# life-ufes/multimodal-model-skin-lesion-classifier

Measured on AMD Instinct MI355X. Metric: images/sec fwd+bwd, ResNet-50+crossattention bs=256, higher is better.
Workload: dtype bf16; 1 GPU; ResNet-50 + one-hot(20) + crossattention, 224x224, train step incl. Adam; per_gpu_batch=256, global_batch=256, parallelism=dp1, weights=random init (torchvision / timm / transformers layouts), unfreeze_weights=unfrozen_weights, linear_dtype=fp32

## Files before the change

include/mmskin.h:

```cpp
#ifndef MMSKIN_H
#define MMSKIN_H
#include <stdint.h>

#ifdef __cplusplus
extern "C" {
#endif

#define MMSKIN_F32 0
#define MMSKIN_BF16 1

const char* mmskin_last_error(void);
int mmskin_version(void);

typedef struct mmskin_backbone* mmskin_backbone_t;
int mmskin_backbone_create(const char* arch, int batch, int height, int width, int dtype, mmskin_backbone_t* out);
void mmskin_backbone_destroy(mmskin_backbone_t h);
int mmskin_backbone_num_tensors(mmskin_backbone_t h, int kind );
int mmskin_backbone_tensor_info(mmskin_backbone_t h, int kind, int index, char* name, int name_cap,
                                int64_t* offset, int64_t* numel, int* ndim, int64_t* shape4);
int64_t mmskin_backbone_param_numel(mmskin_backbone_t h);
int64_t mmskin_backbone_buffer_numel(mmskin_backbone_t h);
int64_t mmskin_backbone_workspace_bytes(mmskin_backbone_t h);
int mmskin_backbone_feature_dim(mmskin_backbone_t h);
int mmskin_backbone_feature_hw(mmskin_backbone_t h, int* out_h, int* out_w);
int mmskin_backbone_num_units(mmskin_backbone_t h);
int mmskin_backbone_unit_info(mmskin_backbone_t h, int index, char* name, int name_cap, int64_t* info12);
int mmskin_backbone_profile_enable(mmskin_backbone_t h, int on);
int mmskin_backbone_profile_read(mmskin_backbone_t h, double* ms7, double* flops7, double* bytes7, int64_t* launches7);
int mmskin_backbone_forward(mmskin_backbone_t h, const float* image_nchw, const float* params, float* buffers,
                            void* workspace, float* features, int training, void* stream);
int mmskin_backbone_forward_u8(mmskin_backbone_t h, const uint8_t* image_nhwc, const float* mean_std6, const float* params,
                               float* buffers, void* workspace, float* features, int training, void* stream);
int mmskin_backbone_set_option(mmskin_backbone_t h, const char* key, int value);
int mmskin_backbone_set_pointer(mmskin_backbone_t h, const char* key, const void* device_ptr);
int mmskin_backbone_num_grad_segments(mmskin_backbone_t h, int* count);
int mmskin_backbone_grad_segment(mmskin_backbone_t h, int index, int64_t* offset, int64_t* numel);
int mmskin_backbone_wait_grad_segment(mmskin_backbone_t h, int index, void* stream);
int mmskin_backbone_last_conv_shape(mmskin_backbone_t h, int* C, int* OH, int* OW);
int mmskin_backbone_last_conv_export(mmskin_backbone_t h, const void* workspace, float* x_nchw, void* stream);
int mmskin_backbone_last_conv_grad(mmskin_backbone_t h, const float* dfeatures, const void* workspace, float* dx_nchw,
                                   void* stream);
int mmskin_backbone_backward(mmskin_backbone_t h, const float* dfeatures, const float* params, void* workspace,
                             float* param_grads, void* stream);

int64_t mmskin_conv2d_workspace_bytes(int N, int Cin, int H, int W, int Cout, int kh, int kw, int stride, int pad);
int mmskin_conv2d_forward(const float* x, const float* w, float* y, int N, int Cin, int H, int W, int Cout, int kh,
                          int kw, int stride, int pad, int dtype, void* workspace, void* stream);
int mmskin_conv2d_backward(const float* dy, const float* x, const float* w, float* dx, float* dw, int N, int Cin,
                           int H, int W, int Cout, int kh, int kw, int stride, int pad, int dtype, void* workspace,
                           void* stream);
int mmskin_conv2d_dgrad_fused_rows(int N, int Cin, int H, int W, int Cout, int kh, int kw, int stride, int pad);
int mmskin_conv2d_dgrad_fused(const float* dy, const float* w, const float* xc, const float* scale, const float* shift, float* dz,
                              float* partial, int* rows_written, int N, int Cin, int H, int W, int Cout, int kh, int kw, int stride,
                              int pad, void* workspace, void* stream);
int64_t mmskin_conv3x3_c64_launches(void);
int64_t mmskin_stem7x7_launches(void);
double mmskin_conv2d_time(int N, int Cin, int H, int W, int Cout, int kh, int kw, int stride, int pad, int dtype,
                          int iters, void* workspace, void* stream);
double mmskin_conv2d_dgrad_time(int N, int Cin, int H, int W, int Cout, int kh, int kw, int stride, int pad, int dtype,
                                int iters, void* workspace, void* stream);
double mmskin_conv2d_wgrad_time(int N, int Cin, int H, int W, int Cout, int kh, int kw, int stride, int pad, int dtype,
                                int iters, void* workspace, void* stream);
int64_t mmskin_conv_pipe_launches(void);
int64_t mmskin_wgrad_ring_launches(void);
int64_t mmskin_wgrad3_ring_launches(void);
int64_t mmskin_abn_workspace_bytes(int N, int Cw, int C4, int H, int W);
int mmskin_abn_backward(const float* g, const float* y, const float* w, const float* cA, const float* cB, const float* cC, int N, int Cw,
                        int C4, int H, int W, float* dy, float* dw, void* workspace, void* stream);
int mmskin_abn_backward_kept_gram(const float* g, const float* y, const float* w, const float* cA, const float* cB, const float* cC, int N,
                                  int Cw, int C4, int H, int W, float* dy, float* dw, void* workspace, void* stream);
int mmskin_conv1x1_gram_stats(const float* y, const float* w, int N, int Cw, int C4, int H, int W, float* stat_sum, float* stat_sq,
                              void* workspace, void* stream);
int64_t mmskin_batchnorm_workspace_bytes(int N, int C, int H, int W);
int mmskin_batchnorm_forward(const float* x, const float* gamma, const float* beta, float* running_mean,
                             float* running_var, float* y, float* save_mean, float* save_invstd, int N, int C, int H,
                             int W, float eps, float momentum, int relu, int dtype, void* workspace, void* stream);
int mmskin_batchnorm_backward(const float* dy, const float* x, const float* gamma, const float* beta,
                              const float* save_mean, const float* save_invstd, float* dx, float* dgamma, float* dbeta,
                              int N, int C, int H, int W, int relu, int dtype, void* workspace, void* stream);
int64_t mmskin_stem_workspace_bytes(int N, int H, int W);
int mmskin_stem_forward(const float* x, const float* w, const float* gamma, const float* beta, float* y, int N, int H,
                        int W, float eps, int dtype, void* workspace, void* stream);
int mmskin_stem_backward(const float* dy, const float* x, const float* w, const float* gamma, const float* beta,
                         float* dw, float* dgamma, float* dbeta, int N, int H, int W, float eps, int dtype,
                         void* workspace, void* stream);

int mmskin_linear_forward(const float* x, const float* w, const float* b, float* y, int M, int K, int N, int relu,
                          void* stream);
int mmskin_linear_backward(const float* dy, const float* x, const float* w, const float* y_relu, float* dy_scratch,
                           float* dx, float* dw, float* db, int M, int K, int N, void* stream);
int mmskin_linear_gelu_backward(const float* dh, const float* x, const float* w, const float* z, float* dy_scratch, float* dx, float* dw,
                                float* db, int M, int K, int N, void* stream);
int mmskin_linear_x16_pitch(int M, int K, int N);
enum { MMSKIN_LINEAR_SMALL = 0, MMSKIN_LINEAR_BIG_F32 = 1, MMSKIN_LINEAR_BIG_BF16 = 2, MMSKIN_LINEAR_PADDED_BF16 = 3 };
int mmskin_linear_route(int M, int K, int N);
int mmskin_linear_forward_keep(const float* x, const float* w, const float* b, const float* res, float* y, void* x16_keep, int M, int K,
                               int N, int relu, void* stream);
int mmskin_linear_backward_keep(const float* dy, const void* x16, const float* w, const float* y_relu, const float* z_gelu, float* dy_scratch,
                                float* dx, float* dw, float* db, int M, int K, int N, void* stream);
int mmskin_gelu_forward_bf16(const float* z, void* h16, int64_t rows, int cols, int cols_pad, void* stream);
int mmskin_linear_forward_x16(const void* x16, const float* w, const float* b, const float* res, float* y, int M, int K, int N, int relu,
                              void* stream);
int mmskin_star_relu_forward_bf16(const float* z, const float* s, const float* b, void* h16, int64_t rows, int cols, int cols_pad,
                                  void* stream);
int mmskin_linear_star_relu_backward_keep(const float* dh, const void* x16, const float* w, const float* z, const float* s, float* dsb,
                                          float* dx, float* dw, float* db, int M, int K, int N, void* stream);
int mmskin_star_relu_forward(const float* z, const float* s, const float* b, float* y, int64_t n, void* stream);
int mmskin_star_relu_backward(const float* dy, const float* z, const float* s, float* dz, float* dsb, int64_t n, void* stream);
int mmskin_layernorm_forward(const float* x, const float* g, const float* b, float* y, float* mean, float* rstd,
                             int M, int N, float eps, int relu, void* stream);
int mmskin_layernorm_backward(const float* dy, const float* x, const float* g, const float* b, const float* mean,
                              const float* rstd, float* dx, float* dg, float* db, int M, int N, int relu, void* stream);
int mmskin_sigmoid_gate_forward(const float* z, const float* v, float* out, int64_t n, void* stream);
int mmskin_sigmoid_gate_backward(const float* dout, const float* z, const float* v, float* dz, float* dv, int64_t n,
                                 void* stream);
int mmskin_gated_mix_forward(const float* z, const float* a, const float* q, float* out, int64_t n, void* stream);
int mmskin_gated_mix_backward(const float* dout, const float* z, const float* a, const float* q, float* dz, float* da,
                              float* dq, int64_t n, void* stream);
int mmskin_metablock_gate_forward(const float* V, const float* t1, const float* t2, float* out, int64_t n, void* stream);
int mmskin_metablock_gate_backward(const float* dout, const float* V, const float* t1, const float* t2, float* dV,
                                   float* dt1, float* dt2, int64_t n, void* stream);
int mmskin_adam_step(float* p, const float* g, float* m, float* v, int64_t n, double lr, double beta1, double beta2, double eps,
                     double weight_decay, int64_t step, void* stream);
int mmskin_dropout_forward(const float* x, float* y, uint8_t* mask, int64_t n, float p, uint64_t seed,
                           uint64_t offset, void* stream);
int mmskin_attn_dropout_forward(const float* x, float* y, uint8_t* mask, int64_t n, int L, float p, uint64_t seed, uint64_t offset,
                                void* stream);
int mmskin_dropout_backward(const float* dy, const uint8_t* mask, float* dx, int64_t n, float p, void* stream);
int mmskin_concat2_forward(const float* a, const float* b, float* out, int M, int Na, int Nb, void* stream);
int mmskin_concat2_backward(const float* dout, float* da, float* db, int M, int Na, int Nb, void* stream);
int mmskin_attention_forward(const float* q, const float* k, const float* v, float* o, float* p, int B, int H, int L,
                             int Dh, float drop_p, uint64_t seed, uint64_t offset, void* stream);
int mmskin_attention_backward(const float* dO, const float* q, const float* k, const float* v, const float* p,
                              float* dq, float* dk, float* dv, int B, int H, int L, int Dh, float drop_p,
                              uint64_t seed, uint64_t offset, void* stream);
int mmskin_mdnet_fuse_forward(const float* feat, const float* z, const float* t1, const float* t2, float* pooled,
                              int64_t NC, int HW, void* stream);
int mmskin_mdnet_fuse_backward(const float* dpooled, const float* feat, const float* z, const float* t1, const float* t2,
                               float* dfeat , float* dz, float* dt1, float* dt2, int64_t NC, int HW,
                               void* stream);
int mmskin_bmm(const float* a, const float* b, float* c, int batch, int M, int N, int K, int64_t sam, int64_t sak, int64_t sab,
               int64_t sbn, int64_t sbk, int64_t sbb, int64_t ldc, int64_t scb, void* stream);
int mmskin_softmax_forward(const float* x, const float* mask_add, const float* bias ,
                           float* y, int64_t rows, int L, int64_t rows_per_batch, float scale,
                           int causal , void* stream);
int mmskin_softmax_backward(const float* dy, const float* y, float* dx, int64_t rows, int L, float scale, void* stream);
int mmskin_colsum(const float* x, float* out, int M, int N, void* stream);
int mmskin_scale_add_forward(const float* x, const float* b, const float* gamma, float* y, int64_t n, int C, void* stream);
int mmskin_scale_mul(const float* dy, const float* v, float* out, int64_t n, int C, int per_channel, void* stream);
int mmskin_token_mean_forward(const float* x, float* out, int B, int L, int E, int start, void* stream);
int mmskin_token_mean_backward(const float* dout, float* dx, int B, int L, int E, int start, void* stream);
int mmskin_flash_attention_forward(const void* q, const void* k, const void* v, const float* mask_add, const float* bias,
                                   void* o, float* lse, int B, int H, int L, int Dh, const int64_t* strides12, int io_dtype,
                                   float scale, int causal, float drop_p, uint64_t seed, uint64_t offset, void* stream);
int mmskin_flash_attention_backward(const float* q, const float* k, const float* v, const float* o, const float* dout, const float* lse,
                                    const float* mask_add, const float* bias, const float* biasT, float* delta, float* dq, float* dk,
                                    float* dv, float* ds_out, int B, int H, int L, int Dh, const int64_t* strides15, float scale,
                                    int causal, float drop_p, uint64_t seed, uint64_t offset, void* stream);
int mmskin_linear_forward_ex(const void* x, int x_dtype, const float* w, const float* b, void* y, int y_dtype, int M, int K, int N,
                             int act, void* stream);
int mmskin_attention_rows_forward(const float* q, const float* k, const float* v, float* o, float* lse, int B, int H, int L, int Dh,
                                  const int64_t* qkv_strides, const int64_t* o_strides, float scale, float drop_p, uint64_t seed,
                                  uint64_t offset, void* stream);
int mmskin_attention_rows_backward(const float* dO, const float* q, const float* k, const float* v, const float* o, const float* lse,
                                   float* dq, float* dk, float* dv, int B, int H, int L, int Dh, const int64_t* qkv_strides,
                                   const int64_t* o_strides, float scale, float drop_p, uint64_t seed, uint64_t offset, void* stream);
int mmskin_window_attention_forward(const float* q, const float* k, const float* v, float* o, float* lse, int B, int nwy, int nwx, int ws,
                                    int H, int Dh, int64_t q_tok, int64_t q_head, int64_t o_tok, int64_t o_head, float scale,
                                    float drop_p, uint64_t seed, uint64_t offset, void* stream);
int mmskin_window_attention_backward(const float* dO, const float* q, const float* k, const float* v, const float* o, const float* lse,
                                     float* dq, float* dk, float* dv, int B, int nwy, int nwx, int ws, int H, int Dh, int64_t q_tok,
                                     int64_t q_head, int64_t o_tok, int64_t o_head, float scale, float drop_p, uint64_t seed,
                                     uint64_t offset, void* stream);
int64_t mmskin_channel_attention_scratch_floats(int B, int G, int N);
int mmskin_channel_attention_forward(const float* q, const float* k, const float* v, float* x, float* attn, float* scratch, int B, int G,
                                     int N, int Dh, int64_t q_tok, int64_t q_b, int64_t o_tok, int64_t o_b, float scale, void* stream);
int mmskin_channel_attention_backward(const float* dO, const float* q, const float* k, const float* v, const float* attn, float* dq,
                                      float* dk, float* dv, float* scratch, int B, int G, int N, int Dh, int64_t q_tok, int64_t q_b,
                                      int64_t o_tok, int64_t o_b, float scale, void* stream);
int mmskin_linear_lane(const void* x, int x_dtype, const void* w, int w_dtype, const float* b, const float* gamma,
                       const float* residual, float drop_p, uint64_t seed, uint64_t offset, void* y, int y_dtype, int M, int K,
                       int N, int act, void* stream);
int mmskin_layernorm_forward_mixed(const float* x, const float* g, const float* b, float* y_f32, void* y_bf16, int M, int N,
                                   float eps, void* stream);
int mmskin_set_linear_dtype(int dtype);
int mmskin_get_linear_dtype(void);
int mmskin_add(const float* a, const float* b, float* y, int64_t n, int64_t nb, void* stream);
int mmskin_gelu_forward(const float* x, float* y, int64_t n, void* stream);
int mmskin_gelu_backward(const float* dy, const float* x, float* dx, int64_t n, void* stream);
int mmskin_gelu_tanh_forward(const float* x, float* y, int64_t n, void* stream);
int mmskin_gelu_tanh_backward(const float* dy, const float* x, float* dx, int64_t n, void* stream);
int64_t mmskin_dwconv3_scratch_floats(int N, int H, int W, int C);
int mmskin_dwconv3_forward(const float* x, const float* w, float* w_stage, float* y, int N, int H, int W, int C, void* stream);
int mmskin_dwconv3_backward(const float* dy, const float* x, const float* w, float* w_stage, float* scratch, float* dx, float* dw,
                            int N, int H, int W, int C, void* stream);
int mmskin_conv_pos_enc_forward(const float* x, const float* w, const float* b, float* w_stage, float* y, int N, int H, int W, int C,
                                void* stream);
int mmskin_conv_pos_enc_backward(const float* dy, const float* x, const float* w, float* w_stage, float* scratch, float* dx, float* dw,
                                 float* db, int N, int H, int W, int C, void* stream);
int64_t mmskin_dw7_star_scratch_floats(int N, int H, int W, int C);
int mmskin_dw7_star_forward(const float* z, const float* w, const float* s, const float* b, float* y, int N, int H, int W, int C,
                            void* stream);
int mmskin_dw7_star_backward(const float* dy, const float* z, const float* w, const float* s, const float* b, float* scratch, float* dz,
                             float* dw, float* dsb, int N, int H, int W, int C, void* stream);
int64_t mmskin_factor_attention_scratch_floats(int B, int H, int W, int Ch, int backward);
int mmskin_factor_attention_forward(const float* qkv, const float* w3, const float* b3, const float* w5, const float* b5, const float* w7,
                                    const float* b7, float* att, float* F, float* stats, float* scratch, int B, int H, int W, int Ch,
                                    void* stream);
int mmskin_factor_attention_backward(const float* dO, const float* qkv, const float* w3, const float* b3, const float* w5, const float* b5,
                                     const float* w7, const float* b7, const float* F, const float* stats, float* dqkv, float* dw3,
                                     float* db3, float* dw5, float* db5, float* dw7, float* db7, float* scratch, int B, int H, int W,
                                     int Ch, void* stream);
int64_t mmskin_conv_pos_enc_tokens_scratch_floats(int B, int H, int W, int C);
int mmskin_conv_pos_enc_tokens_forward(const float* x, const float* w, const float* b, float* y, int B, int H, int W, int C, void* stream);
int mmskin_conv_pos_enc_tokens_backward(const float* dy, const float* x, const float* w, float* scratch, float* dx, float* dw, float* db, int B,
                                        int H, int W, int C, void* stream);
int mmskin_embedding_forward(const float* table, const int64_t* ids, float* out, int B, int ncols, int card, int E,
                             void* stream);
int mmskin_embedding_backward(const float* dout, const int64_t* ids, float* dtable, int B, int ncols, int card, int E,
                              void* stream);

int mmskin_im2col_forward(const float* x, int N, int C, int H, int W, int k, int stride, int pad, int channels_last, float* cols,
                          void* stream);
int mmskin_im2col_backward(const float* dcols, int N, int C, int H, int W, int k, int stride, int pad, int channels_last, float* dx,
                           void* stream);
int mmskin_resize_u8(const uint8_t* src_nhwc, int N, int src_h, int src_w, uint8_t* dst_nhwc, int dst_h, int dst_w,
                     void* stream);
int mmskin_metadata_encode(const int32_t* codes, int n_cat, const int32_t* col_offset, int onehot_width, const float* numeric,
                           int n_num, const float* mean, const float* scale, float nan_fill, float* out, int batch, void* stream);

int mmskin_direct_conv2d_forward(const float* x, const float* w, const float* b, float* y, int N, int Cin, int H, int W,
                                 int Cout, int kh, int kw, int stride, int pad, int relu, void* stream);
int mmskin_direct_conv2d_backward(const float* dy, const float* x, const float* y_relu, float* dw, float* db, int N,
                                  int Cin, int H, int W, int Cout, int kh, int kw, int stride, int pad, void* stream);
int mmskin_pool_gap_forward(const float* x, float* y, int32_t* idx, int N, int C, int H, int W, int k, void* stream);
int mmskin_pool_gap_backward(const float* dy, const int32_t* idx, float* dx, int N, int C, int H, int W, int k,
                             void* stream);

#ifdef __cplusplus
}
#endif
#endif
```

multimodal-model-skin-lesion-classifier_amd/csrc/backbone.hip:

```cpp
#include "plan.h"

namespace {

struct Unit {
  ConvShape s;
  bool stem = false;
  int64_t w_off, g_off, b_off;
  int64_t rm_off, rv_off;
  int64_t wf_off, wd_off;
  size_t x_off;
  size_t y_off;
  size_t coef_off;
  bool abn = false;
  size_t gram_off = 0;
  bool fwd2p = false;
  size_t abn_coef_off = 0;
  size_t rows() const { return (size_t)s.N * s.OH() * s.OW(); }
};

struct Block {
  std::vector<int> units;
  int ds = -1;
  size_t mask_off = 0;
  size_t in_off;
  int in_C, in_H, in_W;
  int seg_done = -1;
};

struct Plan : PlanBase {
  int arch;
  int Hp, Wp, OH0, OW0, PH, PW;
  std::vector<Unit> units;
  std::vector<Block> blocks;
  int64_t staged_elems = 0;
  size_t off_img4, off_wf, off_wd, off_stat, off_pool, off_idx, off_scratch[7], off_slab, off_partial,
      off_coefbwd, off_dwv, off_red, off_partial_b, off_stat_b, off_red_b;
  size_t off_abn_wd = 0, off_abn_bias = 0, off_abn_S = 0, off_abn_cs = 0;
  size_t off_abn_wd2 = 0, off_abn_bias2 = 0;
  size_t off_abn_sgx = 0, off_abn_slab2 = 0, off_abn_S2 = 0, off_abn_cs2 = 0;
  size_t maxact_bytes = 0, stat_bytes = 0;

  int forward(const void* image, const float* norm6, const float* params, float* buffers, unsigned char* ws,
              float* features, bool training, hipStream_t st) override;
  int backward(const float* dfeat, const float* params, unsigned char* ws, float* grads, hipStream_t st) override;
  int last_conv_shape(int* C, int* OH, int* OW) const override;
  int last_conv_export(const unsigned char* ws, float* x_nchw, hipStream_t st) override;
  int last_conv_grad(const float* dfeat, const unsigned char* ws, float* dx_nchw, hipStream_t st) override;
  int num_units() const override { return (int)units.size(); }
  int unit_info(int index, std::string* name, int64_t* info12) const override;
};

int add_unit(Plan& p, const std::string& conv_name, const std::string& bn_name, ConvShape s) {
  Unit u;
  u.s = s;
  u.w_off = add_tensor(p.params, p.param_numel, conv_name + ".weight", {s.Cout, s.Cin, s.kh, s.kw});
  u.g_off = add_tensor(p.params, p.param_numel, bn_name + ".weight", {s.Cout});
  u.b_off = add_tensor(p.params, p.param_numel, bn_name + ".bias", {s.Cout});
  u.rm_off = add_tensor(p.buffers, p.buffer_numel, bn_name + ".running_mean", {s.Cout});
  u.rv_off = add_tensor(p.buffers, p.buffer_numel, bn_name + ".running_var", {s.Cout});
  p.units.push_back(u);
  return (int)p.units.size() - 1;
}

int build_plan(Plan& p) {
  const bool bottleneck = p.arch == 50;
  const int depths18[4] = {2, 2, 2, 2}, depths50[4] = {3, 4, 6, 3};
  const int* depths = bottleneck ? depths50 : depths18;
  const int expansion = bottleneck ? 4 : 1;
  ConvShape s0 = {p.N, p.H, p.W, 3, 64, 7, 7, 2, 3};
  int u0 = add_unit(p, "conv1", "bn1", s0);
  p.units[u0].stem = true;
  p.OH0 = s0.OH(); p.OW0 = s0.OW();
  p.Hp = 2 * p.OH0 + 8; p.Wp = 2 * p.OW0 + 8;
  if (p.Hp < p.H + 6) p.Hp = p.H + 6;
  if (p.Wp < p.W + 6) p.Wp = p.W + 6;
  p.Wp = (p.Wp + 1) / 2 * 2;
  p.PH = (p.OH0 + 2 - 3) / 2 + 1; p.PW = (p.OW0 + 2 - 3) / 2 + 1;
  int cin = 64, h = p.PH, w = p.PW;
  const int widths[4] = {64, 128, 256, 512};
  std::vector<int64_t> seg_starts;
  for (int li = 0; li < 4; ++li) {
    for (int b = 0; b < depths[li]; ++b) {
      const int stride = (b == 0 && li > 0) ? 2 : 1;
      const int width = widths[li], cout = width * expansion;
      std::string base = "layer" + std::to_string(li + 1) + "." + std::to_string(b);
      Block blk;
      blk.in_C = cin; blk.in_H = h; blk.in_W = w;
      if (bottleneck) {
        blk.units.push_back(add_unit(p, base + ".conv1", base + ".bn1", {p.N, h, w, cin, width, 1, 1, 1, 0}));
        blk.units.push_back(add_unit(p, base + ".conv2", base + ".bn2", {p.N, h, w, width, width, 3, 3, stride, 1}));
        int h2 = (h + 2 - 3) / stride + 1, w2 = (w + 2 - 3) / stride + 1;
        blk.units.push_back(add_unit(p, base + ".conv3", base + ".bn3", {p.N, h2, w2, width, cout, 1, 1, 1, 0}));
      } else {
        blk.units.push_back(add_unit(p, base + ".conv1", base + ".bn1", {p.N, h, w, cin, width, 3, 3, stride, 1}));
        int h2 = (h + 2 - 3) / stride + 1, w2 = (w + 2 - 3) / stride + 1;
        blk.units.push_back(add_unit(p, base + ".conv2", base + ".bn2", {p.N, h2, w2, width, cout, 3, 3, 1, 1}));
      }
      if (stride != 1 || cin != cout)
        blk.ds = add_unit(p, base + ".downsample.0", base + ".downsample.1", {p.N, h, w, cin, cout, 1, 1, stride, 0});
      if (b == 0 && li > 0) {
        blk.seg_done = 3 - li;
        seg_starts.push_back(p.units[blk.units[0]].w_off);
      }
      p.blocks.push_back(blk);
      cin = cout;
      h = (h + 2 - 3) / stride + 1;
      w = (w + 2 - 3) / stride + 1;
    }
  }
  p.feat_dim = cin;
  {
    int64_t end = p.param_numel;
    for (int i = 2; i >= 0; --i) {
      PlanBase::GradSegment g;
      g.offset = seg_starts[i]; g.numel = end - seg_starts[i];
      p.segments.push_back(g);
      end = seg_starts[i];
    }
    PlanBase::GradSegment g;
    g.offset = 0; g.numel = end;
    p.segments.push_back(g);
  }

  std::vector<StageDesc> table;
  int64_t wf = 0, wd = 0;
  for (Unit& u : p.units) {
    StageDesc d = {};
    d.src_off = u.w_off;
    d.Cout = u.s.Cout; d.Cin = u.s.Cin; d.taps = u.s.kh * u.s.kw; d.stem = u.stem ? 1 : 0;
    u.wf_off = wf; u.wd_off = wd;
    d.fwd_off = wf; d.dgrad_off = wd;
    int64_t n = u.stem ? 64 * 256 : (int64_t)d.Cout * d.Cin * d.taps;
    wf += n;
    if (!u.stem) wd += n;
    if (d.Cout * d.Cin * d.taps > p.max_stage_elems) p.max_stage_elems = d.Cout * d.Cin * d.taps;
    table.push_back(d);
  }
  p.staged_elems = wf;
  p.table_host = table;

  const size_t es = p.esz();
  size_t cur = 0;
  p.off_img4 = carve(cur, (size_t)p.N * p.Hp * p.Wp * 4 * es);
  p.off_wf = carve(cur, (size_t)wf * es);
  p.off_wd = carve(cur, (size_t)wd * es);
  size_t stat_rows_max = 0, maxact = 0, slab_max = stem_wgrad_slab_bytes(p.N, p.OH0, p.OW0), partial_max = 0;
  int maxC = 64;
  for (Unit& u : p.units) {
    size_t rows = u.rows();
    size_t sr = (size_t)ceil_div((int)rows, 128) * u.s.Cout;
    if (sr > stat_rows_max) stat_rows_max = sr;
    if (rows * u.s.Cout > maxact) maxact = rows * u.s.Cout;
    if ((size_t)u.s.N * u.s.H * u.s.W * u.s.Cin > maxact && !u.stem) maxact = (size_t)u.s.N * u.s.H * u.s.W * u.s.Cin;
    if (!u.stem) { size_t sb = conv_wgrad_slab_bytes(u.s); if (sb > slab_max) slab_max = sb; }
    size_t pr = (size_t)bn_bwd_partial_rows(rows, u.s.Cout) * 2 * u.s.Cout * sizeof(float);
    if (pr > partial_max) partial_max = pr;
    pr = ((rows + 127) / 128 + 4) * 2 * u.s.Cout * sizeof(float);
    if (pr > partial_max) partial_max = pr;
    if (u.s.Cout > maxC) maxC = u.s.Cout;
  }
  p.stat_bytes = stat_rows_max * sizeof(float);
  p.off_stat = carve(cur, 2 * p.stat_bytes);
  p.off_stat_b = carve(cur, 2 * p.stat_bytes);
  p.maxact_bytes = maxact * es;
  for (Unit& u : p.units) {
    u.coef_off = carve(cur, 4 * (size_t)u.s.Cout * sizeof(float));
    u.x_off = carve(cur, u.rows() * u.s.Cout * es);
  }
  for (size_t i = 0; i < p.units.size(); ++i) {
    StageDesc& d = p.table_host[i];
    const Unit& u = p.units[i];
    d.has_bn = 1;
    d.bn_g_off = u.g_off; d.bn_b_off = u.b_off; d.bn_rm_off = u.rm_off; d.bn_rv_off = u.rv_off;
    d.coef_off = (int64_t)u.coef_off;
  }
  p.off_pool = carve(cur, (size_t)p.N * p.PH * p.PW * 64 * es);
  p.off_idx = carve(cur, (size_t)p.N * p.PH * p.PW * 64);
  size_t prev = p.off_pool;
  for (Block& b : p.blocks) {
    b.in_off = prev;
    for (int ui : b.units) {
      Unit& u = p.units[ui];
      u.y_off = carve(cur, u.rows() * u.s.Cout * es);
    }
    prev = p.units[b.units.back()].y_off;
    Unit& bl = p.units[b.units.back()];
    b.mask_off = carve(cur, bl.rows() * bl.s.Cout * es / 16);
  }
  for (int i = 0; i < 7; ++i) p.off_scratch[i] = carve(cur, p.maxact_bytes);
  {
    constexpr int abn_maxc = 128;
    size_t wd_max = 0, s_max = 0;
    int cw_max = 0;
    std::vector<int> cand;
    for (Block& b : p.blocks) { cand.push_back(b.units.back()); if (b.ds >= 0) cand.push_back(b.ds); }
    for (int ui : cand) {
      Unit& u = p.units[ui];
      WgradRingPlan rp;
      int sh = 0;
      while ((u.s.Cin << sh) < u.s.Cout) ++sh;
      if (p.dtype != 1 || !bottleneck || u.s.kh != 1 || u.s.stride != 1 || u.s.Cin > abn_maxc || u.s.Cin % 64 || (u.s.Cin << sh) != u.s.Cout ||
          !wgrad_gram_plan((int)u.rows(), u.s.Cout, u.s.Cin, rp) || rp.gram_tiles != 1)
        continue;
      u.abn = true;
      u.abn_coef_off = carve(cur, 3 * (size_t)u.s.Cout * sizeof(float));
      const size_t sb = wgrad_gram_slab_bytes((int)u.rows(), u.s.Cout, u.s.Cin);
      if (sb > slab_max) slab_max = sb;
      const size_t wdb = (size_t)u.s.Cin * (u.s.Cout + u.s.Cin) * 2, sf = ((size_t)u.s.Cout + 64 * rp.wo) * u.s.Cin * sizeof(float);
      if (wdb > wd_max) wd_max = wdb;
      if (sf > s_max) s_max = sf;
      if (u.s.Cin > cw_max) cw_max = u.s.Cin;
    }
    if (wd_max) {
      p.off_abn_wd = carve(cur, wd_max);
      p.off_abn_bias = carve(cur, (size_t)cw_max * sizeof(float));
      p.off_abn_S = carve(cur, s_max);
      p.off_abn_cs = carve(cur, (size_t)cw_max * sizeof(float));
      p.off_abn_wd2 = carve(cur, wd_max);
      p.off_abn_bias2 = carve(cur, (size_t)cw_max * sizeof(float));
      size_t slab2 = 0;
      for (Block& b : p.blocks) {
        Unit& u = p.units[b.units.back()];
        if (!u.abn || b.ds >= 0) continue;
        u.fwd2p = true;
        size_t sb = wgrad_gram_slab_bytes((int)u.rows(), u.s.Cout, u.s.Cin);
        if (sb > slab2) slab2 = sb;
        WgradRingPlan rg;
        if (wgrad_gram_plan((int)u.rows(), 0, u.s.Cin, rg, 2) && rg.gram_tiles == 1 &&
            wgrad_gram_slab_bytes((int)u.rows(), u.s.Cout, u.s.Cin, 1)) {
          u.gram_off = carve(cur, ((size_t)128 + 1) * u.s.Cin * sizeof(float));
          sb = wgrad_gram_slab_bytes((int)u.rows(), 0, u.s.Cin, 2);
          if (sb > slab2) slab2 = sb;
          sb = wgrad_gram_slab_bytes((int)u.rows(), u.s.Cout, u.s.Cin, 1);
          if (sb > slab2) slab2 = sb;
        }
      }
      if (slab2) {
        p.off_abn_sgx = carve(cur, 1024 * sizeof(float));
        p.off_abn_slab2 = carve(cur, slab2);
        p.off_abn_S2 = carve(cur, s_max);
        p.off_abn_cs2 = carve(cur, (size_t)cw_max * sizeof(float));
      }
    }
  }
  p.off_slab = carve(cur, slab_max);
  p.off_partial = carve(cur, partial_max);
  p.off_partial_b = carve(cur, partial_max);
  p.off_coefbwd = carve(cur, 3 * (size_t)maxC * sizeof(float));
  p.off_dwv = carve(cur, 64 * 256 * sizeof(float));
  p.off_red = carve(cur, bn_reduce_scratch_bytes(maxC));
  p.off_red_b = carve(cur, bn_reduce_scratch_bytes(maxC));
  p.ws_bytes = cur;
  return MMSKIN_OK;
}

template <typename T>
int forward_eval(Plan& p, const void* image, const float* norm6, const float* params, float* buffers, unsigned char* ws,
                 float* features, hipStream_t st, bool reuse_table) {
  const float eps = 1e-5f;
  T* wf = reinterpret_cast<T*>(ws + p.off_wf);
  int rc, maxC = 64;
  for (const Unit& u : p.units) maxC = u.s.Cout > maxC ? u.s.Cout : maxC;
  if (!reuse_table) PROF(K_BN_FWD, 0.0, 0.0, bn_eval_table(p.table_dev, (int)p.units.size(), maxC, params, buffers, ws, eps, st));
  auto shift_of = [&](const Unit& u) { return reinterpret_cast<const float*>(ws + u.coef_off) + u.s.Cout; };
  Unit& u0 = p.units[0];
  T* img4 = reinterpret_cast<T*>(ws + p.off_img4);
  if (norm6) PROF(K_STEM_MISC, 0.0, 0.0, stem_pack_u8<T>((const uint8_t*)image, p.N, p.H, p.W, p.Hp, p.Wp, norm6, img4, st));
  else PROF(K_STEM_MISC, 0.0, 0.0, stem_pack<T>((const float*)image, p.N, p.H, p.W, p.Hp, p.Wp, img4, st));
  T* x0 = reinterpret_cast<T*>(ws + u0.x_off);
  PROF(K_CONV_FWD, conv_flops(u0.s), conv_bytes(u0.s, sizeof(T)),
       launch_stem_conv_fwd<T>(p.N, p.OH0, p.OW0, p.Hp, p.Wp, img4, wf + u0.wf_off, x0, nullptr, nullptr, st));
  const float* c0 = reinterpret_cast<const float*>(ws + u0.coef_off);
  T* pool = reinterpret_cast<T*>(ws + p.off_pool);
  PROF(K_STEM_MISC, 0.0, 0.0, stem_bn_relu_pool<T>(x0, c0, c0 + 64, p.N, p.OH0, p.OW0, 64, pool, ws + p.off_idx, st));
  for (Block& b : p.blocks) {
    const T* in = reinterpret_cast<const T*>(ws + b.in_off);
    const T* cur = in;
    const int nu = (int)b.units.size();
    const T* skip = in;
    if (b.ds >= 0) {
      Unit& d = p.units[b.ds];
      FwdFuse f; f.bias = shift_of(d);
      T* xd = reinterpret_cast<T*>(ws + d.x_off);
      PROF(K_CONV_FWD, conv_flops(d.s), conv_bytes(d.s, sizeof(T)), launch_conv_fwd<T>(d.s, in, wf + d.wf_off, xd, nullptr, nullptr, st, &f));
      skip = xd;
    }
    for (int i = 0; i < nu; ++i) {
      Unit& u = p.units[b.units[i]];
      T* y = reinterpret_cast<T*>(ws + u.y_off);
      FwdFuse f; f.bias = shift_of(u); f.relu = true;
      if (i + 1 == nu) f.addend = skip;
      PROF(K_CONV_FWD, conv_flops(u.s), conv_bytes(u.s, sizeof(T), 0), launch_conv_fwd<T>(u.s, cur, wf + u.wf_off, y, nullptr, nullptr, st, &f));
      cur = y;
    }
  }
  Unit& last = p.units[p.blocks.back().units.back()];
  return avgpool_fwd<T>(reinterpret_cast<const T*>(ws + last.y_off), p.N, last.s.OH() * last.s.OW(), last.s.Cout, features, st);
}

template <typename T>
int forward_impl(Plan& p, const void* image, const float* norm6, const float* params, float* buffers, unsigned char* ws,
                 float* features, bool training, hipStream_t st) {
  const float eps = 1e-5f, mom = 0.1f;
  T* wf = reinterpret_cast<T*>(ws + p.off_wf);
  T* wd = reinterpret_cast<T*>(ws + p.off_wd);
  float* stat_sum = reinterpret_cast<float*>(ws + p.off_stat);
  float* stat_sq = reinterpret_cast<float*>(ws + p.off_stat + p.stat_bytes);
  int rc;
  if ((rc = p.ensure_table())) return rc;
  const bool folded_eval = !training && !p.keep_raw_eval;
  const bool reuse = folded_eval && p.reuse_staged && p.staged_eval_ws == ws;
  p.staged_eval_ws = folded_eval ? ws : nullptr;
  if (!reuse) HIP_CHECK_RET(hipMemsetAsync(wf + p.units[0].wf_off, 0, 64 * 256 * sizeof(T), st));
  const bool use_side = !p.prof.on;
  if (use_side && (rc = p.side.init())) return rc;
  const bool stage_aside = use_side && training;
  const float* fold = (training || p.keep_raw_eval) ? nullptr : buffers;
  if (stage_aside) {
    if ((rc = stage_weights<T>(p.table_dev, 1, p.max_stage_elems, params, wf, wd, training, st, fold, eps))) return rc;
    HIP_CHECK_RET(hipEventRecord(p.side.f_ready, st));
    HIP_CHECK_RET(hipStreamWaitEvent(p.side.s, p.side.f_ready, 0));
    if ((rc = stage_weights<T>(p.table_dev + 1, (int)p.units.size() - 1, p.max_stage_elems, params, wf, wd, training, p.side.s,
                               fold, eps))) return rc;
    HIP_CHECK_RET(hipEventRecord(p.side.f_staged, p.side.s));
  } else if (!reuse) {
    PROF(K_STAGE, 0.0, 0.0, stage_weights<T>(p.table_dev, (int)p.units.size(), p.max_stage_elems, params, wf, wd, training, st, fold, eps));
  }
  if (folded_eval) return forward_eval<T>(p, image, norm6, params, buffers, ws, features, st, reuse);

  auto bn_coeffs_on = [&](Unit& u, int stat_rows, float* ssum, float* ssq, double* red, hipStream_t s2) -> int {
    float* coef = reinterpret_cast<float*>(ws + u.coef_off);
    const int C = u.s.Cout;
    p.prof.begin(K_BN_FWD, s2);
    struct End { Profiler& pr; hipStream_t s; ~End() { pr.end(s); } } end_guard{p.prof, s2};
    if (training)
      return bn_finalize(ssum, ssq, stat_rows, C, (double)u.rows(), params + u.g_off, params + u.b_off, eps,
                         mom, buffers + u.rm_off, buffers + u.rv_off, coef, coef + C, coef + 2 * C, coef + 3 * C, red, s2);
    return bn_eval_coeffs(C, params + u.g_off, params + u.b_off, buffers + u.rm_off, buffers + u.rv_off, eps, coef,
                          coef + C, s2);
  };
  auto bn_coeffs = [&](Unit& u, int stat_rows) -> int {
    return bn_coeffs_on(u, stat_rows, stat_sum, stat_sq, reinterpret_cast<double*>(ws + p.off_red), st);
  };
  float* stat_b_sum = reinterpret_cast<float*>(ws + p.off_stat_b);
  float* stat_b_sq = reinterpret_cast<float*>(ws + p.off_stat_b + p.stat_bytes);

  Unit& u0 = p.units[0];
  T* img4 = reinterpret_cast<T*>(ws + p.off_img4);
  if (norm6) PROF(K_STEM_MISC, 0.0, 0.0, stem_pack_u8<T>((const uint8_t*)image, p.N, p.H, p.W, p.Hp, p.Wp, norm6, img4, st));
  else PROF(K_STEM_MISC, 0.0, 0.0, stem_pack<T>((const float*)image, p.N, p.H, p.W, p.Hp, p.Wp, img4, st));
  T* x0 = reinterpret_cast<T*>(ws + u0.x_off);
  int stem_rows = 0;
  PROF(K_CONV_FWD, conv_flops(u0.s), conv_bytes(u0.s, sizeof(T)),
       launch_stem_conv_fwd<T>(p.N, p.OH0, p.OW0, p.Hp, p.Wp, img4, wf + u0.wf_off, x0,
                               training ? stat_sum : nullptr, training ? stat_sq : nullptr, st, &stem_rows));
  if ((rc = bn_coeffs(u0, stem_rows))) return rc;
  float* c0 = reinterpret_cast<float*>(ws + u0.coef_off);
  T* pool = reinterpret_cast<T*>(ws + p.off_pool);
  PROF(K_STEM_MISC, 0.0, 0.0, stem_bn_relu_pool<T>(x0, c0, c0 + 64, p.N, p.OH0, p.OW0, 64, pool, ws + p.off_idx, st));

  if (stage_aside) HIP_CHECK_RET(hipStreamWaitEvent(st, p.side.f_staged, 0));
  for (Block& b : p.blocks) {
    const T* in = reinterpret_cast<const T*>(ws + b.in_off);
    const T* cur = in;
    const int nu = (int)b.units.size();
    if (b.ds >= 0) {
      Unit& d = p.units[b.ds];
      if (use_side) {
        HIP_CHECK_RET(hipEventRecord(p.side.f_ready, st));
        HIP_CHECK_RET(hipStreamWaitEvent(p.side.s, p.side.f_ready, 0));
        int nrows_d = 0;
        if ((rc = launch_conv_fwd<T>(d.s, in, wf + d.wf_off, reinterpret_cast<T*>(ws + d.x_off),
                                     training ? stat_b_sum : nullptr, training ? stat_b_sq : nullptr, p.side.s, nullptr, &nrows_d))) return rc;
        if ((rc = bn_coeffs_on(d, nrows_d, stat_b_sum, stat_b_sq,
                               reinterpret_cast<double*>(ws + p.off_red_b), p.side.s))) return rc;
        HIP_CHECK_RET(hipEventRecord(p.side.f_done, p.side.s));
      } else {
        int nrows_d = 0;
        PROF(K_CONV_FWD, conv_flops(d.s), conv_bytes(d.s, sizeof(T)),
             launch_conv_fwd<T>(d.s, in, wf + d.wf_off, reinterpret_cast<T*>(ws + d.x_off),
                                training ? stat_sum : nullptr, training ? stat_sq : nullptr, st, nullptr, &nrows_d));
        if ((rc = bn_coeffs(d, nrows_d))) return rc;
      }
    }
    for (int i = 0; i < nu; ++i) {
      Unit& u = p.units[b.units[i]];
      T* x = reinterpret_cast<T*>(ws + u.x_off);
      T* y = reinterpret_cast<T*>(ws + u.y_off);
      int nrows_u = 0;
      const bool two_pass = training && u.fwd2p && i + 1 == nu && sizeof(T) == 2;
      const bool gram_pass = two_pass && u.gram_off != 0;
      if (gram_pass) {
        if constexpr (sizeof(T) == 2) {
          float* gm = reinterpret_cast<float*>(ws + u.gram_off);
          float* gcs = gm + (size_t)128 * u.s.Cin;
          PROF(K_BN_FWD, 0.0, (double)u.rows() * u.s.Cin * sizeof(T),
               launch_wgrad_gram(u.s.N, u.s.OH(), u.s.OW(), u.s.Cin, u.s.Cout, nullptr, cur, reinterpret_cast<float*>(ws + p.off_abn_slab2), gm, gcs, st, 2));
          float* cf = reinterpret_cast<float*>(ws + u.coef_off);
          const int Cq = u.s.Cout;
          PROF(K_BN_FWD, 0.0, 0.0, gram_stats_finalize(gm, gcs, params + u.w_off, Cq, u.s.Cin, (double)u.rows(), params + u.g_off, params + u.b_off, eps, mom,
                                                       buffers + u.rm_off, buffers + u.rv_off, cf, cf + Cq, cf + 2 * Cq, cf + 3 * Cq, st));
          nrows_u = -1;
        }
      } else {
        PROF(K_CONV_FWD, conv_flops(u.s), conv_bytes(u.s, sizeof(T)),
             launch_conv_fwd<T>(u.s, cur, wf + u.wf_off, two_pass ? (T*)nullptr : x, training ? stat_sum : nullptr,
                                training ? stat_sq : nullptr, st, nullptr, &nrows_u));
      }
      if (nrows_u >= 0 && (rc = bn_coeffs(u, nrows_u))) return rc;
      float* coef = reinterpret_cast<float*>(ws + u.coef_off);
      const int C = u.s.Cout;
      if (two_pass) {
        FwdFuse f2; f2.mul = coef; f2.bias = coef + C; f2.addend = in; f2.relu = true; f2.mask_out = ws + b.mask_off;
        PROF(K_CONV_FWD, gram_pass ? conv_flops(u.s) : 0.0, conv_bytes(u.s, sizeof(T), 0) + (double)u.rows() * C * sizeof(T), launch_conv_fwd<T>(u.s, cur, wf + u.wf_off, y, nullptr, nullptr, st, &f2));
      } else if (i + 1 < nu) {
        PROF(K_BN_FWD, 0.0, 2.0 * u.rows() * C * sizeof(T), bn_apply<T>(x, nullptr, coef, coef + C, nullptr, nullptr, y, u.rows(), C, true, st));
      } else if (b.ds >= 0) {
        Unit& d = p.units[b.ds];
        float* dc = reinterpret_cast<float*>(ws + d.coef_off);
        if (use_side) HIP_CHECK_RET(hipStreamWaitEvent(st, p.side.f_done, 0));
        PROF(K_BN_FWD, 0.0, 3.0 * u.rows() * C * sizeof(T),
             bn_apply<T>(x, reinterpret_cast<const T*>(ws + d.x_off), coef, coef + C, dc, dc + C, y, u.rows(), C, true, st,
                         training ? ws + b.mask_off : nullptr));
      } else {
        PROF(K_BN_FWD, 0.0, 3.0 * u.rows() * C * sizeof(T),
             bn_apply<T>(x, in, coef, coef + C, nullptr, nullptr, y, u.rows(), C, true, st, training ? ws + b.mask_off : nullptr));
      }
      cur = y;
    }
  }
  Unit& last = p.units[p.blocks.back().units.back()];
  return avgpool_fwd<T>(reinterpret_cast<const T*>(ws + last.y_off), p.N, last.s.OH() * last.s.OW(), last.s.Cout,
                        features, st);
}

template <typename T>
int backward_impl(Plan& p, const float* dfeat, const float* params, unsigned char* ws, float* grads,
                  hipStream_t st) {
  T* wd = reinterpret_cast<T*>(ws + p.off_wd);
  float* slab = reinterpret_cast<float*>(ws + p.off_slab);
  float* partial = reinterpret_cast<float*>(ws + p.off_partial);
  float* cA = reinterpret_cast<float*>(ws + p.off_coefbwd);
  T* S[7];
  for (int i = 0; i < 7; ++i) S[i] = reinterpret_cast<T*>(ws + p.off_scratch[i]);
  int rc;

  auto bn_backward = [&](Unit& u, const T* dy, const T* ymask, int mode, T* dx, T* dz) -> int {
    const int C = u.s.Cout;
    float* coef = reinterpret_cast<float*>(ws + u.coef_off);
    const T* x = reinterpret_cast<const T*>(ws + u.x_off);
    float* cB = cA + C; float* cC = cA + 2 * C;
    int r, nr = 0;
    p.prof.begin(K_BN_BWD, st);
    struct End { Profiler& pr; hipStream_t s; ~End() { pr.end(s); } } end_guard{p.prof, st};
    if (p.prof.on) p.prof.bytes[K_BN_BWD] += (mode == MASK_FROM_Y ? 7.0 : 5.0) * u.rows() * C * sizeof(T);
    if ((r = bn_bwd_reduce<T>(dy, x, ymask, coef, coef + C, mode, u.rows(), C, partial, &nr, st))) return r;
    if ((r = bn_bwd_finalize(partial, nr, C, (double)u.rows(), params + u.g_off,
                             coef + 2 * C, coef + 3 * C, grads + u.g_off, grads + u.b_off, cA, cB, cC,
                             reinterpret_cast<double*>(ws + p.off_red), st))) return r;
    return bn_bwd_apply<T>(dy, x, ymask, coef, coef + C, mode, cA, cB, cC, dx, dz, u.rows(), C, st);
  };

  float* partial_b = reinterpret_cast<float*>(ws + p.off_partial_b);
  auto bn_backward_fused = [&](Unit& u, const T* dz, const float* part, int nrows, T* dx, const float* sum_dz_x = nullptr) -> int {
    const int C = u.s.Cout;
    float* coef = reinterpret_cast<float*>(ws + u.coef_off);
    const T* x = reinterpret_cast<const T*>(ws + u.x_off);
    float* cB = cA + C; float* cC = cA + 2 * C;
    double* red = reinterpret_cast<double*>(ws + p.off_red);
    int r;
    p.prof.begin(K_BN_BWD, st);
    struct End { Profiler& pr; hipStream_t s; ~End() { pr.end(s); } } end_guard{p.prof, st};
    if (p.prof.on && dx) p.prof.bytes[K_BN_BWD] += 3.0 * u.rows() * C * sizeof(T);
    if ((r = bn_bwd_finalize(part, nrows, C, (double)u.rows(), params + u.g_off, coef + 2 * C, coef + 3 * C,
                             grads + u.g_off, grads + u.b_off, cA, cB, cC, red, st, -1, false, sum_dz_x))) return r;
    if (!dx) return MMSKIN_OK;
    return bn_bwd_apply<T>(dz, x, nullptr, coef, coef + C, MASK_NONE, cA, cB, cC, dx, nullptr, u.rows(), C, st);
  };

  Unit& last = p.units[p.blocks.back().units.back()];
  T* g = S[0];
  T* gin = S[1];
  if ((rc = avgpool_bwd<T>(dfeat, p.N, last.s.OH() * last.s.OW(), last.s.Cout, g, st))) return rc;

  const bool use_side = !p.prof.on;
  if (use_side && (rc = p.side.init())) return rc;
  for (int i = 0; i < 3; ++i) p.side.done_valid[i] = false;
  T* DX[3] = {S[2], S[6], S[5]};
  auto acquire = [&](int i) -> int {
    if (use_side && p.side.done_valid[i]) HIP_CHECK_RET(hipStreamWaitEvent(st, p.side.done[i], 0));
    return MMSKIN_OK;
  };
  auto wgrad_async = [&](Unit& u, int i, const T* uin) -> int {
    hipStream_t ws_st = st;
    if (use_side) {
      HIP_CHECK_RET(hipEventRecord(p.side.ready[i], st));
      HIP_CHECK_RET(hipStreamWaitEvent(p.side.s, p.side.ready[i], 0));
      ws_st = p.side.s;
    }
    p.prof.begin(K_WGRAD, st);
    int r = launch_conv_wgrad<T>(u.s, DX[i], uin, slab, grads + u.w_off, ws_st);
    p.prof.end(st);
    if (p.prof.on) { p.prof.flops[K_WGRAD] += conv_flops(u.s); p.prof.bytes[K_WGRAD] += conv_bytes(u.s, sizeof(T)); }
    if (r) return r;
    if (use_side) {
      HIP_CHECK_RET(hipEventRecord(p.side.done[i], p.side.s));
      p.side.done_valid[i] = true;
    }
    return MMSKIN_OK;
  };
  int dxi = 0;
  for (int i = 0; i < 2; ++i) p.side.g_done_valid[i] = false;
  auto g_index = [&](const T* buf) { return buf == S[0] ? 0 : 1; };
  auto g_acquire = [&](const T* buf) -> int {
    const int i = g_index(buf);
    if (use_side && p.side.g_done_valid[i]) HIP_CHECK_RET(hipStreamWaitEvent(st, p.side.g_done[i], 0));
    return MMSKIN_OK;
  };
  auto wgrad_abn_async = [&](Unit& u, const T* gbuf, const T* uin) -> int {
    if constexpr (sizeof(T) == 2) {
      hipStream_t ws_st = st;
      if (use_side) {
        HIP_CHECK_RET(hipEventRecord(p.side.g_ready, st));
        HIP_CHECK_RET(hipStreamWaitEvent(p.side.s, p.side.g_ready, 0));
        ws_st = p.side.s;
      }
      float* S_out = reinterpret_cast<float*>(ws + p.off_abn_S);
      float* cs_out = reinterpret_cast<float*>(ws + p.off_abn_cs);
      p.prof.begin(K_WGRAD, st);
      int r = launch_wgrad_gram(u.s.N, u.s.OH(), u.s.OW(), u.s.Cin, u.s.Cout, gbuf, uin, slab, S_out, cs_out, ws_st);
      if (!r) r = abn_wgrad_finalize(S_out, cs_out, params + u.w_off, reinterpret_cast<const float*>(ws + u.abn_coef_off), u.s.Cout, u.s.Cin,
                                     grads + u.w_off, ws_st);
      p.prof.end(st);
      if (p.prof.on) { p.prof.flops[K_WGRAD] += conv_flops(u.s); p.prof.bytes[K_WGRAD] += conv_bytes(u.s, sizeof(T)); }
      if (r) return r;
      if (use_side) {
        const int gi = g_index(gbuf);
        HIP_CHECK_RET(hipEventRecord(p.side.g_done[gi], p.side.s));
        p.side.g_done_valid[gi] = true;
      }
      return MMSKIN_OK;
    } else {
      return MMSKIN_ERR_UNSUPPORTED;
    }
  };

  bool fused_ready = false;
  int fused_rows = 0;
  for (int bi = (int)p.blocks.size() - 1; bi >= 0; --bi) {
    Block& b = p.blocks[bi];
    const int nu = (int)b.units.size();
    const T* in = reinterpret_cast<const T*>(ws + b.in_off);
    Unit& ul = p.units[b.units[nu - 1]];
    const T* out = reinterpret_cast<const T*>(ws + ul.y_off);
    T* dY = S[3];
    T* dZ = S[4];
    T* dXd = DX[2];
    const bool has_ds = b.ds >= 0;
    const T* dz_final;
    dxi ^= 1;
    if ((rc = acquire(dxi))) return rc;
    if (has_ds && (rc = acquire(2))) return rc;
    T* dX = DX[dxi];
    const bool abn = fused_ready && ul.abn && sizeof(T) == 2;
    if (fused_ready) {
      const T* uin3 = nu > 1 ? reinterpret_cast<const T*>(ws + p.units[b.units[nu - 2]].y_off) : in;
      const float* sgx = nullptr;
      if (abn && ul.fwd2p) {
        if constexpr (sizeof(T) == 2) {
          float* S2 = reinterpret_cast<float*>(ws + p.off_abn_S2);
          p.prof.begin(K_WGRAD, st);
          rc = launch_wgrad_gram(ul.s.N, ul.s.OH(), ul.s.OW(), ul.s.Cin, ul.s.Cout, g, uin3, reinterpret_cast<float*>(ws + p.off_abn_slab2), S2,
                                 reinterpret_cast<float*>(ws + p.off_abn_cs2), st, ul.gram_off ? 1 : 0);
          p.prof.end(st);
          if (p.prof.on) { p.prof.flops[K_WGRAD] += conv_flops(ul.s); p.prof.bytes[K_WGRAD] += conv_bytes(ul.s, sizeof(T)); }
          if (rc) return rc;
          if ((rc = abn_sgx(S2, params + ul.w_off, ul.s.Cout, ul.s.Cin, reinterpret_cast<float*>(ws + p.off_abn_sgx), st))) return rc;
          sgx = reinterpret_cast<const float*>(ws + p.off_abn_sgx);
        }
      }
      if ((rc = bn_backward_fused(ul, g, partial, fused_rows, abn ? nullptr : dX, sgx))) return rc;
      if (abn) {
        if constexpr (sizeof(T) == 2) {
          if ((rc = abn_prep(params + ul.w_off, cA, cA + ul.s.Cout, cA + 2 * ul.s.Cout, ul.s.Cout, ul.s.Cin, reinterpret_cast<bf16_t*>(ws + p.off_abn_wd),
                             reinterpret_cast<float*>(ws + p.off_abn_bias), reinterpret_cast<float*>(ws + ul.abn_coef_off), st))) return rc;
          const float* gkept = ul.gram_off ? reinterpret_cast<const float*>(ws + ul.gram_off) : nullptr;
          if (ul.fwd2p && (rc = abn_wgrad_finalize(reinterpret_cast<const float*>(ws + p.off_abn_S2),
                                                   gkept ? gkept + (size_t)128 * ul.s.Cin : reinterpret_cast<const float*>(ws + p.off_abn_cs2), params + ul.w_off,
                                                   reinterpret_cast<const float*>(ws + ul.abn_coef_off), ul.s.Cout, ul.s.Cin, grads + ul.w_off, st, gkept))) return rc;
        }
      }
      if (has_ds) {
        Unit& d = p.units[b.ds];
        const bool abn_d = d.abn && sizeof(T) == 2;
        if ((rc = bn_backward_fused(d, g, partial_b, fused_rows, abn_d ? nullptr : dXd))) return rc;
        if (abn_d) {
          if constexpr (sizeof(T) == 2) {
            if ((rc = abn_prep(params + d.w_off, cA, cA + d.s.Cout, cA + 2 * d.s.Cout, d.s.Cout, d.s.Cin, reinterpret_cast<bf16_t*>(ws + p.off_abn_wd2),
                               reinterpret_cast<float*>(ws + p.off_abn_bias2), reinterpret_cast<float*>(ws + d.abn_coef_off), st))) return rc;
          }
        }
      }
      dz_final = g;
    } else {
      if ((rc = bn_backward(ul, g, out, MASK_FROM_Y, dX, has_ds ? nullptr : dZ))) return rc;
      if (has_ds)
        if ((rc = bn_backward(p.units[b.ds], g, out, MASK_FROM_Y, dXd, nullptr))) return rc;
      dz_final = dZ;
    }
    for (int i = nu - 1; i >= 0; --i) {
      Unit& u = p.units[b.units[i]];
      const T* uin = i == 0 ? in : reinterpret_cast<const T*>(ws + p.units[b.units[i - 1]].y_off);
      const bool abn_u = abn && i == nu - 1;
      if (abn_u) { if (!u.fwd2p && (rc = wgrad_abn_async(u, g, uin))) return rc; }
      else if ((rc = wgrad_async(u, dxi, uin))) return rc;
      if (i > 0) {
        Unit& up = p.units[b.units[i - 1]];
        float* cup = reinterpret_cast<float*>(ws + up.coef_off);
        DgradFuse f;
        f.x = ws + up.x_off; f.scale = cup; f.shift = cup + up.s.Cout; f.partial = partial;
        if (abn_u) {
          f.in2 = uin; f.k2 = u.s.Cin; f.bias = reinterpret_cast<const float*>(ws + p.off_abn_bias);
          PROF(K_CONV_DGRAD, conv_flops(u.s), conv_bytes(u.s, sizeof(T), 1), launch_conv_dgrad<T>(u.s, g, reinterpret_cast<const T*>(ws + p.off_abn_wd), dY, (const T*)nullptr, st, &f));
        } else
        PROF(K_CONV_DGRAD, conv_flops(u.s), conv_bytes(u.s, sizeof(T), 1), launch_conv_dgrad<T>(u.s, dX, wd + u.wd_off, dY, (const T*)nullptr, st, &f));
        dxi ^= 1;
        if ((rc = acquire(dxi))) return rc;
        dX = DX[dxi];
        if ((rc = bn_backward_fused(up, dY, partial, f.rows_written, dX))) return rc;
      } else {
        const T* addend = dz_final;
        bool ds_addend_compact = false;
        static const bool ds_compact = env_knob("MMSKIN_DS_COMPACT", 1) != 0;
        if (has_ds) {
          Unit& d = p.units[b.ds];
          if ((rc = g_acquire(gin))) return rc;
          if (fused_ready && d.abn && sizeof(T) == 2) {
            if ((rc = wgrad_abn_async(d, g, in))) return rc;
            DgradFuse fd;
            fd.in2 = in; fd.k2 = d.s.Cin; fd.bias = reinterpret_cast<const float*>(ws + p.off_abn_bias2);
            PROF(K_CONV_DGRAD, conv_flops(d.s), conv_bytes(d.s, sizeof(T)), launch_conv_dgrad<T>(d.s, g, reinterpret_cast<const T*>(ws + p.off_abn_wd2), gin, (const T*)nullptr, st, &fd));
          } else if (ds_compact && bi > 0 && d.s.kh == 1 && d.s.stride == 2 && d.s.pad == 0 && u.s.kh == 1 && u.s.stride == 1) {
            if ((rc = wgrad_async(d, 2, in))) return rc;
            ConvShape dc = d.s;
            dc.H = d.s.OH(); dc.W = d.s.OW(); dc.stride = 1;
            PROF(K_CONV_DGRAD, conv_flops(d.s), conv_bytes(d.s, sizeof(T)), launch_conv_dgrad<T>(dc, dXd, wd + d.wd_off, S[3], (const T*)nullptr, st));
            ds_addend_compact = true;
          } else {
            if ((rc = wgrad_async(d, 2, in))) return rc;
            PROF(K_CONV_DGRAD, conv_flops(d.s), conv_bytes(d.s, sizeof(T)), launch_conv_dgrad<T>(d.s, dXd, wd + d.wd_off, gin, (const T*)nullptr, st));
          }
          addend = ds_addend_compact ? S[3] : gin;
        }
        if ((rc = g_acquire(gin))) return rc;
        DgradFuse f;
        DgradFuse* fp = nullptr;
        if (bi > 0) {
          Block& pb = p.blocks[bi - 1];
          Unit& pu = p.units[pb.units.back()];
          f.mask_bits = ws + pb.mask_off; f.x = pu.fwd2p ? nullptr : ws + pu.x_off; f.partial = partial;
          if (pb.ds >= 0) { f.x2 = ws + p.units[pb.ds].x_off; f.partial_b = partial_b; }
          f.addend_s2 = ds_addend_compact;
          fp = &f;
        }
        PROF(K_CONV_DGRAD, conv_flops(u.s), conv_bytes(u.s, sizeof(T), 1 + (fp ? (f.x2 ? 3 : 2) : 0)), launch_conv_dgrad<T>(u.s, dX, wd + u.wd_off, gin, addend, st, fp));
        fused_ready = fp != nullptr;
        fused_rows = f.rows_written;
      }
    }
    T* t = g; g = gin; gin = t;
    if (b.seg_done >= 0 && (rc = p.segment_done(b.seg_done, st, use_side))) return rc;
  }

  Unit& u0 = p.units[0];
  T* dx0 = S[3];
  {
    float* c0 = reinterpret_cast<float*>(ws + u0.coef_off);
    const T* x0 = reinterpret_cast<const T*>(ws + u0.x_off);
    float* cB = cA + 64; float* cC = cA + 128;
    int nr = 0;
    p.prof.begin(K_BN_BWD, st);
    if (stem_sums_pooled()) rc = stem_pool_bwd_sums<T>(g, reinterpret_cast<const T*>(ws + p.off_pool), ws + p.off_idx, x0, c0, c0 + 64, p.N, p.OH0, p.OW0, 64, partial, &nr, st);
    else rc = stem_pool_bn_bwd_reduce<T>(g, ws + p.off_idx, x0, c0, c0 + 64, p.N, p.OH0, p.OW0, 64, partial, &nr, st);
    if (!rc) rc = bn_bwd_finalize(partial, nr, 64, (double)u0.rows(), params + u0.g_off, c0 + 128, c0 + 192, grads + u0.g_off,
                                  grads + u0.b_off, cA, cB, cC, reinterpret_cast<double*>(ws + p.off_red), st);
    if (!rc) rc = stem_pool_bn_bwd_apply<T>(g, ws + p.off_idx, x0, c0, c0 + 64, cA, cB, cC, p.N, p.OH0, p.OW0, 64, dx0, st);
    p.prof.end(st);
    if (p.prof.on) p.prof.bytes[K_BN_BWD] += 3.5 * u0.rows() * 64 * sizeof(T);
    if (rc) return rc;
  }
  float* dwv = reinterpret_cast<float*>(ws + p.off_dwv);
  hipStream_t wst = st;
  if (use_side) {
    HIP_CHECK_RET(hipEventRecord(p.side.ready[0], st));
    HIP_CHECK_RET(hipStreamWaitEvent(p.side.s, p.side.ready[0], 0));
    wst = p.side.s;
  }
  p.prof.begin(K_WGRAD, st);
  rc = launch_stem_conv_wgrad<T>(p.N, p.OH0, p.OW0, p.Hp, p.Wp, dx0, reinterpret_cast<const T*>(ws + p.off_img4), slab, dwv, wst);
  p.prof.end(st);
  if (p.prof.on) p.prof.flops[K_WGRAD] += conv_flops(u0.s);
  if (rc) return rc;
  if ((rc = stem_wgrad_unpack(dwv, grads + u0.w_off, wst))) return rc;
  if (use_side) {
    HIP_CHECK_RET(hipEventRecord(p.side.done[0], p.side.s));
    HIP_CHECK_RET(hipStreamWaitEvent(st, p.side.done[0], 0));
  }
  return p.segment_done((int)p.segments.size() - 1, st, false);
}

int Plan::forward(const void* image, const float* norm6, const float* params, float* buffers, unsigned char* ws,
                  float* features, bool training, hipStream_t st) {
  if (dtype == 1) return forward_impl<bf16_t>(*this, image, norm6, params, buffers, ws, features, training, st);
  return forward_impl<float>(*this, image, norm6, params, buffers, ws, features, training, st);
}
int Plan::backward(const float* dfeat, const float* params, unsigned char* ws, float* grads, hipStream_t st) {
  if (dtype == 1) return backward_impl<bf16_t>(*this, dfeat, params, ws, grads, st);
  return backward_impl<float>(*this, dfeat, params, ws, grads, st);
}
int Plan::last_conv_shape(int* C, int* OH, int* OW) const {
  const Unit& u = units[blocks.back().units.back()];
  *C = u.s.Cout; *OH = u.s.OH(); *OW = u.s.OW();
  return MMSKIN_OK;
}
int Plan::last_conv_export(const unsigned char* ws, float* x_nchw, hipStream_t st) {
  const Unit& u = units[blocks.back().units.back()];
  if (dtype == 1) return nhwc_to_nchw<bf16_t>(reinterpret_cast<const bf16_t*>(ws + u.x_off), N, u.s.Cout, u.s.OH(), u.s.OW(), x_nchw, st);
  return nhwc_to_nchw<float>(reinterpret_cast<const float*>(ws + u.x_off), N, u.s.Cout, u.s.OH(), u.s.OW(), x_nchw, st);
}
int Plan::last_conv_grad(const float* dfeat, const unsigned char* ws, float* dx_nchw, hipStream_t st) {
  const Unit& u = units[blocks.back().units.back()];
  const float* scale = reinterpret_cast<const float*>(ws + u.coef_off);
  const int HW = u.s.OH() * u.s.OW();
  if (dtype == 1) return gap_relu_bn_grad<bf16_t>(dfeat, reinterpret_cast<const bf16_t*>(ws + u.y_off), scale, N, HW, u.s.Cout, dx_nchw, st);
  return gap_relu_bn_grad<float>(dfeat, reinterpret_cast<const float*>(ws + u.y_off), scale, N, HW, u.s.Cout, dx_nchw, st);
}
int Plan::unit_info(int index, std::string* name, int64_t* info12) const {
  const Unit& u = units[index];
  for (const TensorInfo& t : params)
    if (t.offset == u.w_off && name) *name = t.name;
  const int64_t v[12] = {(int64_t)u.x_off, (int64_t)u.y_off, (int64_t)u.coef_off, (int64_t)u.rows(), u.s.Cout,
                         u.s.OH(), u.s.OW(), u.s.Cin, u.s.H, u.s.W, (int64_t)off_pool, (int64_t)off_scratch[0]};
  for (int i = 0; i < 12; ++i) info12[i] = v[i];
  return MMSKIN_OK;
}

}

PlanBase* make_resnet_plan(int arch, int N, int H, int W, int dtype, int* rc) {
  Plan* p = new Plan();
  p->arch = arch; p->N = N; p->H = H; p->W = W; p->dtype = dtype;
  *rc = build_plan(*p);
  if (*rc) { delete p; return nullptr; }
  return p;
}

#include "../../include/mmskin.h"

struct mmskin_backbone { PlanBase* plan = nullptr; };

extern "C" {

int mmskin_backbone_create(const char* arch, int batch, int height, int width, int dtype, mmskin_backbone_t* out) {
  ARG_CHECK(arch && out, "backbone_create: null argument");
  int a = 0;
  if (!strcmp(arch, "resnet-18")) a = 18;
  else if (!strcmp(arch, "resnet-50")) a = 50;
  else if (!strcmp(arch, "densenet169")) a = 169;
  else if (!strcmp(arch, "densenet169-features")) a = 1690;
  else if (!strcmp(arch, "vgg16-features")) a = 16;
  else if (!strcmp(arch, "mobilenet-v2")) a = 2;
  else if (!strcmp(arch, "efficientnet-b0")) a = 100;
  else if (!strcmp(arch, "efficientnet-b7")) a = 107;
  else { mmskin_set_error("backbone_create: Backbone '%s' has no HIP plan", arch); return MMSKIN_ERR_UNSUPPORTED; }
  ARG_CHECK(batch > 0 && height >= 32 && width >= 32, "backbone_create: bad shape %dx%dx%d", batch, height, width);
  ARG_CHECK(dtype == MMSKIN_F32 || dtype == MMSKIN_BF16, "backbone_create: dtype %d", dtype);
  int rc = MMSKIN_OK;
  PlanBase* p = (a == 169 || a == 1690) ? make_densenet_plan(batch, height, width, dtype, a == 1690, &rc)
                : a == 16               ? make_vgg_plan(batch, height, width, dtype, &rc)
                : a == 2                ? make_mobilenet_plan(batch, height, width, dtype, &rc)
                : a >= 100              ? make_efficientnet_plan(a - 100, batch, height, width, dtype, &rc)
                                        : make_resnet_plan(a, batch, height, width, dtype, &rc);
  if (!p) return rc ? rc : MMSKIN_ERR_ARG;
  mmskin_backbone* h = new mmskin_backbone();
  h->plan = p;
  *out = h;
  return MMSKIN_OK;
}

void mmskin_backbone_destroy(mmskin_backbone_t h) {
  if (!h) return;
  delete h->plan;
  delete h;
}

int mmskin_backbone_num_tensors(mmskin_backbone_t h, int kind) {
  return (int)(kind == 0 ? h->plan->params.size() : h->plan->buffers.size());
}

int mmskin_backbone_tensor_info(mmskin_backbone_t h, int kind, int index, char* name, int name_cap,
                                int64_t* offset, int64_t* numel, int* ndim, int64_t* shape4) {
  const std::vector<TensorInfo>& v = kind == 0 ? h->plan->params : h->plan->buffers;
  ARG_CHECK(index >= 0 && index < (int)v.size(), "tensor_info: index %d out of range", index);
  const TensorInfo& t = v[index];
  if (name && name_cap > 0) { strncpy(name, t.name.c_str(), name_cap - 1); name[name_cap - 1] = 0; }
  if (offset) *offset = t.offset;
  if (numel) *numel = t.numel;
  if (ndim) *ndim = t.ndim;
  if (shape4) for (int i = 0; i < 4; ++i) shape4[i] = t.shape[i];
  return MMSKIN_OK;
}

int64_t mmskin_backbone_param_numel(mmskin_backbone_t h) { return h->plan->param_numel; }
int64_t mmskin_backbone_buffer_numel(mmskin_backbone_t h) { return h->plan->buffer_numel; }
int64_t mmskin_backbone_workspace_bytes(mmskin_backbone_t h) { return (int64_t)h->plan->ws_bytes; }
int mmskin_backbone_feature_dim(mmskin_backbone_t h) { return h->plan->feat_dim; }
int mmskin_backbone_feature_hw(mmskin_backbone_t h, int* out_h, int* out_w) {
  ARG_CHECK(h && out_h && out_w, "backbone_feature_hw: null argument");
  *out_h = h->plan->out_h; *out_w = h->plan->out_w;
  return MMSKIN_OK;
}

int mmskin_backbone_profile_enable(mmskin_backbone_t h, int on) {
  h->plan->prof.on = on != 0;
  h->plan->prof.reset();
  return MMSKIN_OK;
}

int mmskin_backbone_profile_read(mmskin_backbone_t h, double* ms7, double* flops7, double* bytes7, int64_t* launches7) {
  Profiler& pr = h->plan->prof;
  HIP_CHECK_RET(hipDeviceSynchronize());
  for (int c = 0; c < K_NCLASS; ++c) { ms7[c] = 0; flops7[c] = pr.flops[c]; bytes7[c] = pr.bytes[c]; launches7[c] = 0; }
  for (size_t i = 0; i < pr.cls.size(); ++i) {
    float ms = 0.f;
    HIP_CHECK_RET(hipEventElapsedTime(&ms, pr.pool[2 * i], pr.pool[2 * i + 1]));
    ms7[pr.cls[i]] += ms;
    launches7[pr.cls[i]] += 1;
  }
  pr.reset();
  return MMSKIN_OK;
}

int mmskin_backbone_num_units(mmskin_backbone_t h) { return h->plan->num_units(); }

int mmskin_backbone_unit_info(mmskin_backbone_t h, int index, char* name, int name_cap, int64_t* info12) {
  ARG_CHECK(index >= 0 && index < h->plan->num_units(), "unit_info: index %d out of range", index);
  std::string nm;
  int rc = h->plan->unit_info(index, &nm, info12);
  if (rc) return rc;
  if (name && name_cap > 0) { strncpy(name, nm.c_str(), name_cap - 1); name[name_cap - 1] = 0; }
  return MMSKIN_OK;
}

int mmskin_backbone_forward(mmskin_backbone_t h, const float* image_nchw, const float* params, float* buffers,
                            void* workspace, float* features, int training, void* stream) {
  ARG_CHECK(h && image_nchw && params && (buffers || h->plan->buffer_numel == 0) && workspace && features, "backbone_forward: null argument");
  return h->plan->forward(image_nchw, nullptr, params, buffers, (unsigned char*)workspace, features, training != 0,
                          (hipStream_t)stream);
}

int mmskin_backbone_forward_u8(mmskin_backbone_t h, const uint8_t* image_nhwc, const float* mean_std6, const float* params,
                               float* buffers, void* workspace, float* features, int training, void* stream) {
  ARG_CHECK(h && image_nhwc && mean_std6 && params && (buffers || h->plan->buffer_numel == 0) && workspace && features, "backbone_forward_u8: null argument");
  return h->plan->forward(image_nhwc, mean_std6, params, buffers, (unsigned char*)workspace, features, training != 0,
                          (hipStream_t)stream);
}

int mmskin_backbone_set_option(mmskin_backbone_t h, const char* key, int value) {
  ARG_CHECK(h && key, "backbone_set_option: null argument");
  if (!strcmp(key, "keep_raw_eval")) { h->plan->keep_raw_eval = value != 0; return MMSKIN_OK; }
  if (!strcmp(key, "reuse_staged")) { h->plan->reuse_staged = value != 0; return MMSKIN_OK; }
  mmskin_set_error("backbone_set_option: unknown option '%s'", key);
  return MMSKIN_ERR_ARG;
}
int mmskin_backbone_num_grad_segments(mmskin_backbone_t h, int* count) {
  ARG_CHECK(h && count, "backbone_num_grad_segments: null argument");
  *count = (int)h->plan->segments.size();
  return MMSKIN_OK;
}
int mmskin_backbone_grad_segment(mmskin_backbone_t h, int index, int64_t* offset, int64_t* numel) {
  ARG_CHECK(h && offset && numel, "backbone_grad_segment: null argument");
  ARG_CHECK(index >= 0 && index < (int)h->plan->segments.size(), "backbone_grad_segment: index %d", index);
  *offset = h->plan->segments[index].offset;
  *numel = h->plan->segments[index].numel;
  return MMSKIN_OK;
}
int mmskin_backbone_wait_grad_segment(mmskin_backbone_t h, int index, void* stream) {
  ARG_CHECK(h, "backbone_wait_grad_segment: null argument");
  ARG_CHECK(index >= 0 && index < (int)h->plan->segments.size(), "backbone_wait_grad_segment: index %d", index);
  int rc = h->plan->segment_wait(index, (hipStream_t)stream);
  if (rc == MMSKIN_ERR_ARG) mmskin_set_error("backbone_wait_grad_segment: no backward has been enqueued on this plan yet");
  return rc;
}
int mmskin_backbone_set_pointer(mmskin_backbone_t h, const char* key, const void* device_ptr) {
  ARG_CHECK(h && key, "backbone_set_pointer: null argument");
  int rc = h->plan->set_pointer(key, device_ptr);
  if (rc) mmskin_set_error("backbone_set_pointer: '%s' is not a pointer this plan takes", key);
  return rc;
}
int mmskin_backbone_last_conv_shape(mmskin_backbone_t h, int* C, int* OH, int* OW) {
  ARG_CHECK(h && C && OH && OW, "backbone_last_conv_shape: null argument");
  int rc = h->plan->last_conv_shape(C, OH, OW);
  if (rc == MMSKIN_ERR_UNSUPPORTED) mmskin_set_error("backbone_last_conv_*: this plan has no Grad-CAM export");
  return rc;
}
int mmskin_backbone_last_conv_export(mmskin_backbone_t h, const void* workspace, float* x_nchw, void* stream) {
  ARG_CHECK(h && workspace && x_nchw, "backbone_last_conv_export: null argument");
  ARG_CHECK(h->plan->keep_raw_eval, "backbone_last_conv_export: set option keep_raw_eval before the forward");
  int rc = h->plan->last_conv_export((const unsigned char*)workspace, x_nchw, (hipStream_t)stream);
  if (rc == MMSKIN_ERR_UNSUPPORTED) mmskin_set_error("backbone_last_conv_*: this plan has no Grad-CAM export");
  return rc;
}
int mmskin_backbone_last_conv_grad(mmskin_backbone_t h, const float* dfeatures, const void* workspace, float* dx_nchw,
                                   void* stream) {
  ARG_CHECK(h && dfeatures && workspace && dx_nchw, "backbone_last_conv_grad: null argument");
  int rc = h->plan->last_conv_grad(dfeatures, (const unsigned char*)workspace, dx_nchw, (hipStream_t)stream);
  if (rc == MMSKIN_ERR_UNSUPPORTED) mmskin_set_error("backbone_last_conv_*: this plan has no Grad-CAM export");
  return rc;
}

int mmskin_backbone_backward(mmskin_backbone_t h, const float* dfeatures, const float* params, void* workspace,
                             float* param_grads, void* stream) {
  ARG_CHECK(h && dfeatures && params && workspace && param_grads, "backbone_backward: null argument");
  return h->plan->backward(dfeatures, params, (unsigned char*)workspace, param_grads, (hipStream_t)stream);
}

}
```

multimodal-model-skin-lesion-classifier_amd/csrc/conv.h:

```cpp
#pragma once
#include "common.h"

struct ConvShape {
  int N, H, W, Cin, Cout, kh, kw, stride, pad;
  int OH() const { return (H + 2 * pad - kh) / stride + 1; }
  int OW() const { return (W + 2 * pad - kw) / stride + 1; }
};

#define MMSKIN_MAX_TAPS 12
struct TapClass {
  int a_dim, b_dim;
  int ph, pw;
  int ntaps;
  int mblk_start;
  int rows;
  int pad_;
  int8_t offy[MMSKIN_MAX_TAPS], offx[MMSKIN_MAX_TAPS], wtap[MMSKIN_MAX_TAPS];
};

struct ConvGemmArgs {
  const void* in;
  const void* w;
  void* out;
  const void* addend;
  float* stat_sum;
  float* stat_sq;
  const void* ep_mask_y;
  const uint8_t* ep_mask_bits;
  const void* ep_x;
  int ep_x_pitch;
  const float* ep_scale;
  const float* ep_shift;
  const float* ep_bias;
  int ep_relu;
  float* out_f32;
  const float* ep_gamma;
  const float* res_f32;
  float ep_drop_p;
  uint64_t ep_seed_mix, ep_offset;
  const void* ep_x2;
  float* stat_b_sum;
  float* stat_b_sq;
  int stat_stride;
  int N, IH, IW, C, Cpitch;
  int Cout, wrow;
  int Sy, Sx, OS;
  int OHf, OWf;
  int ncls, total_mblk, nblk_n;
  int simple_src;
  uint64_t in_bytes;
  int bm_step;
  int pipe_ok;
  int group_m;
  const void* in2;
  int K1, pitch2_shift;
  int addend_sub;
  const float* ep_mul;
  uint8_t* ep_mask_out;
  int ablate;
#ifdef MMSKIN_ABLATE
  unsigned long long* stamps;
#endif
  TapClass cls[4];
};

struct WgradArgs {
  const void* dy;
  const void* in;
  float* slab;
  int N, IH, IW, C, Cpitch;
  int OH, OW;
  int Cout, Ktot;
  int Sy, Sx;
  int ntaps;
  int M, m_per_split, nsplit;
  int nblk_o, nblk_k;
  int simple1x1;
  int nblk_o_main, gram_cols;
  float* colsum;
  int ablate;
  int8_t offy[MMSKIN_MAX_TAPS], offx[MMSKIN_MAX_TAPS];
};

struct WgradRingPlan { int wo, wk, nsplit, mps; bool s1; int gram_tiles; };
bool wgrad_ring_tile(int M, int Cout, int Ktot, WgradRingPlan& r, bool simple);
bool wgrad_ring_plan(const WgradArgs& a, WgradRingPlan& r);
int wgrad_ring_launch(WgradArgs& a, const WgradRingPlan& r, hipStream_t st);
int wgrad_ring_launch_count();
bool wgrad_gram_plan(int M, int Cout, int Cin, WgradRingPlan& r, int mode = 0);
size_t wgrad_gram_slab_bytes(int M, int Cout, int Cin, int mode = 0);
int launch_wgrad_gram(int N, int H, int W, int Cin, int Cout, const bf16_t* g, const bf16_t* in, float* slab, float* s_out, float* colsum_out,
                      hipStream_t st, int mode = 0);

struct FwdFuse {
  const float* bias = nullptr;
  const void* addend = nullptr;
  bool relu = false;
  bool gelu = false;
  float* out_f32 = nullptr;
  const float* gamma = nullptr;
  const float* res_f32 = nullptr;
  float drop_p = 0.f;
  uint64_t seed = 0, offset = 0;
  uint8_t* mask_out = nullptr;
  const float* mul = nullptr;
};
template <typename T>
int launch_conv_fwd(const ConvShape& s, const T* in, const T* w_staged, T* out, float* stat_sum,
                    float* stat_sq, hipStream_t st, const FwdFuse* fuse = nullptr, int* stat_rows_out = nullptr);
int conv_fwd_stat_rows(const ConvShape& s);

struct DgradFuse {
  const void* mask_y = nullptr;
  const uint8_t* mask_bits = nullptr;
  const void* x = nullptr;
  int x_pitch = 0;
  const float* scale = nullptr;
  const float* shift = nullptr;
  const void* x2 = nullptr;
  float* partial = nullptr;
  float* partial_b = nullptr;
  int rows_written = 0;
  const void* in2 = nullptr;
  int k2 = 0;
  const float* bias = nullptr;
  bool addend_s2 = false;
};
int conv_dgrad_partial_rows(const ConvShape& s);

template <typename T>
int launch_conv_dgrad(const ConvShape& s, const T* dout, const T* wt_staged, T* din, const T* addend,
                      hipStream_t st, DgradFuse* fuse = nullptr);

template <typename T>
int launch_stem_conv_fwd(int N, int OH, int OW, int Hp, int Wp, const T* img4, const T* wv, T* out,
                         float* stat_sum, float* stat_sq, hipStream_t st, int* stat_rows_out = nullptr);
int stem_conv_stat_rows(int N, int OH, int OW);
bool stem7x7_takes(int OH, int OW, int Hp, int Wp);
int stem7x7_stat_rows(int N, int OH);
int launch_stem7x7_fwd(int N, int OH, int OW, int Hp, int Wp, const bf16_t* img4, const bf16_t* wv, bf16_t* out, float* stat_sum, float* stat_sq,
                       hipStream_t st);

template <typename T>
int launch_vgg_first_conv_fwd(int N, int H, int W, int Hp, int Wp, const T* img8, const T* wv, T* out,
                              const FwdFuse* fuse, hipStream_t st, int stride = 1, float* stat_sum = nullptr,
                              float* stat_sq = nullptr);
size_t vgg_first_wgrad_slab_bytes(int N, int H, int W);
template <typename T>
int launch_vgg_first_conv_wgrad(int N, int H, int W, int Hp, int Wp, const T* dout, const T* img8, float* slab,
                                float* dwv, hipStream_t st, int stride = 1);

bool conv3x3_c64_takes(const ConvShape& s, bool bf16);
int launch_conv3x3_c64_fwd(const ConvShape& s, const bf16_t* in, const bf16_t* w_staged, bf16_t* out, float* stat_sum, float* stat_sq,
                           int stat_stride, hipStream_t st);
int launch_conv3x3_c64_dgrad(const ConvShape& s, const bf16_t* dout, const bf16_t* wt_staged, bf16_t* din, DgradFuse* fuse, hipStream_t st);

size_t conv_wgrad_slab_bytes(const ConvShape& s);
template <typename T>
int launch_conv_wgrad(const ConvShape& s, const T* dout, const T* in, float* slab, float* dw,
                      hipStream_t st, int cout_valid = 0, int cin_valid = 0);
size_t stem_wgrad_slab_bytes(int N, int OH, int OW);
template <typename T>
int launch_stem_conv_wgrad(int N, int OH, int OW, int Hp, int Wp, const T* dout, const T* img4,
                           float* slab, float* dwv, hipStream_t st);

bool wgrad3_ring_takes(const ConvShape& s, int* nsplit);
int launch_wgrad3_ring(const ConvShape& s, const bf16_t* dout, const bf16_t* in, float* slab, hipStream_t st, int* nsplit);

int abn_prep(const float* W, const float* cA, const float* cB, const float* cC, int C4, int Cw, bf16_t* wd, float* bias, float* coef_copy,
             hipStream_t st);
int abn_wgrad_finalize(const float* S, const float* colsum, const float* W, const float* coef, int C4, int Cw, float* dW, hipStream_t st,
                       const float* gram = nullptr);
int gram_stats(const float* gram, const float* colsum, const float* W, int C4, int Cw, float* stat_sum, float* stat_sq, hipStream_t st);
int gram_stats_finalize(const float* gram, const float* colsum, const float* W, int C4, int Cw, double count, const float* gamma, const float* beta, float eps,
                        float momentum, float* running_mean, float* running_var, float* scale, float* shift, float* save_mean, float* save_invstd,
                        hipStream_t st);
int abn_sgx(const float* S, const float* W, int C4, int Cw, float* sgx, hipStream_t st);
```

multimodal-model-skin-lesion-classifier_amd/csrc/plan.h:

```cpp
#pragma once
#include <stdlib.h>
#include <string.h>

#include <string>
#include <vector>

#include "conv.h"
#include "ops.h"

struct TensorInfo {
  std::string name;
  int64_t offset, numel;
  int ndim;
  int64_t shape[4];
};

enum KClass { K_CONV_FWD = 0, K_CONV_DGRAD, K_WGRAD, K_BN_FWD, K_BN_BWD, K_STAGE, K_STEM_MISC, K_NCLASS };

struct Profiler {
  bool on = false;
  std::vector<hipEvent_t> pool;
  std::vector<int> cls;
  size_t used = 0;
  double flops[K_NCLASS] = {0};
  double bytes[K_NCLASS] = {0};
  hipEvent_t get() {
    if (used == pool.size()) { hipEvent_t e; (void)hipEventCreate(&e); pool.push_back(e); }
    return pool[used++];
  }
  void begin(int c, hipStream_t st) { if (on) { cls.push_back(c); (void)hipEventRecord(get(), st); } }
  void end(hipStream_t st) { if (on) (void)hipEventRecord(get(), st); }
  void reset() { used = 0; cls.clear(); for (int i = 0; i < K_NCLASS; ++i) { flops[i] = 0; bytes[i] = 0; } }
};

struct SideStream {
  hipStream_t s = nullptr;
  hipEvent_t ready[3] = {nullptr, nullptr, nullptr};
  hipEvent_t done[3] = {nullptr, nullptr, nullptr};
  bool done_valid[3] = {false, false, false};
  hipEvent_t f_ready = nullptr, f_done = nullptr;
  hipEvent_t f_staged = nullptr;
  hipEvent_t g_ready = nullptr, g_done[2] = {nullptr, nullptr};
  bool g_done_valid[2] = {false, false};
  int init() {
    if (s) return MMSKIN_OK;
    HIP_CHECK_RET(hipStreamCreateWithFlags(&s, hipStreamNonBlocking));
    for (int i = 0; i < 3; ++i) {
      HIP_CHECK_RET(hipEventCreateWithFlags(&ready[i], hipEventDisableTiming));
      HIP_CHECK_RET(hipEventCreateWithFlags(&done[i], hipEventDisableTiming));
    }
    HIP_CHECK_RET(hipEventCreateWithFlags(&f_ready, hipEventDisableTiming));
    HIP_CHECK_RET(hipEventCreateWithFlags(&f_done, hipEventDisableTiming));
    HIP_CHECK_RET(hipEventCreateWithFlags(&f_staged, hipEventDisableTiming));
    HIP_CHECK_RET(hipEventCreateWithFlags(&g_ready, hipEventDisableTiming));
    HIP_CHECK_RET(hipEventCreateWithFlags(&g_done[0], hipEventDisableTiming));
    HIP_CHECK_RET(hipEventCreateWithFlags(&g_done[1], hipEventDisableTiming));
    return MMSKIN_OK;
  }
  void destroy() {
    if (!s) return;
    for (int i = 0; i < 3; ++i) { (void)hipEventDestroy(ready[i]); (void)hipEventDestroy(done[i]); }
    (void)hipEventDestroy(f_ready); (void)hipEventDestroy(f_done); (void)hipEventDestroy(f_staged);
    if (g_ready) { (void)hipEventDestroy(g_ready); (void)hipEventDestroy(g_done[0]); (void)hipEventDestroy(g_done[1]); }
    (void)hipStreamDestroy(s);
    s = nullptr;
  }
};

struct PlanBase {
  Profiler prof;
  SideStream side;
  int N = 0, H = 0, W = 0, dtype = 0;
  int feat_dim = 0;
  int out_h = 1, out_w = 1;
  std::vector<TensorInfo> params, buffers;
  int64_t param_numel = 0, buffer_numel = 0;
  StageDesc* table_dev = nullptr;
  std::vector<StageDesc> table_host;
  int max_stage_elems = 0;
  size_t ws_bytes = 0;
  size_t esz() const { return dtype == 1 ? 2 : 4; }

  struct GradSegment {
    int64_t offset = 0, numel = 0;
    hipEvent_t ev_main = nullptr, ev_side = nullptr;
    bool side_valid = false;
  };
  std::vector<GradSegment> segments;
  int segment_done(int i, hipStream_t st, bool use_side) {
    GradSegment& g = segments[i];
    if (!g.ev_main) {
      HIP_CHECK_RET(hipEventCreateWithFlags(&g.ev_main, hipEventDisableTiming));
      HIP_CHECK_RET(hipEventCreateWithFlags(&g.ev_side, hipEventDisableTiming));
    }
    HIP_CHECK_RET(hipEventRecord(g.ev_main, st));
    g.side_valid = use_side;
    if (use_side) HIP_CHECK_RET(hipEventRecord(g.ev_side, side.s));
    return MMSKIN_OK;
  }
  int segment_wait(int i, hipStream_t waiter) {
    GradSegment& g = segments[i];
    if (!g.ev_main) return MMSKIN_ERR_ARG;
    HIP_CHECK_RET(hipStreamWaitEvent(waiter, g.ev_main, 0));
    if (g.side_valid) HIP_CHECK_RET(hipStreamWaitEvent(waiter, g.ev_side, 0));
    return MMSKIN_OK;
  }

  virtual ~PlanBase() {
    if (table_dev) (void)hipFree(table_dev);
    for (GradSegment& g : segments)
      if (g.ev_main) { (void)hipEventDestroy(g.ev_main); (void)hipEventDestroy(g.ev_side); }
    side.destroy();
  }
  virtual int forward(const void* image, const float* norm6, const float* params, float* buffers, unsigned char* ws,
                      float* features, bool training, hipStream_t st) = 0;
  virtual int backward(const float* dfeat, const float* params, unsigned char* ws, float* grads, hipStream_t st) = 0;
  bool keep_raw_eval = false;
  bool reuse_staged = false;
  const void* staged_eval_ws = nullptr;
  virtual int last_conv_shape(int*, int*, int*) const { return MMSKIN_ERR_UNSUPPORTED; }
  virtual int last_conv_export(const unsigned char*, float*, hipStream_t) { return MMSKIN_ERR_UNSUPPORTED; }
  virtual int last_conv_grad(const float*, const unsigned char*, float*, hipStream_t) { return MMSKIN_ERR_UNSUPPORTED; }
  virtual int set_pointer(const char*, const void*) { return MMSKIN_ERR_UNSUPPORTED; }
  virtual int num_units() const { return 0; }
  virtual int unit_info(int, std::string*, int64_t*) const { return MMSKIN_ERR_UNSUPPORTED; }

  int ensure_table() {
    if (table_dev) return MMSKIN_OK;
    HIP_CHECK_RET(hipMalloc((void**)&table_dev, table_host.size() * sizeof(StageDesc)));
    HIP_CHECK_RET(hipMemcpy(table_dev, table_host.data(), table_host.size() * sizeof(StageDesc),
                            hipMemcpyHostToDevice));
    return MMSKIN_OK;
  }
};

static inline int64_t add_tensor(std::vector<TensorInfo>& v, int64_t& total, const std::string& name,
                                 std::initializer_list<int64_t> shape) {
  TensorInfo t;
  t.name = name;
  t.offset = total;
  t.ndim = (int)shape.size();
  t.numel = 1;
  int i = 0;
  for (int64_t d : shape) { t.shape[i++] = d; t.numel *= d; }
  for (; i < 4; ++i) t.shape[i] = 1;
  total += t.numel;
  v.push_back(t);
  return t.offset;
}

struct BNRef {
  int64_t g_off, b_off, rm_off, rv_off;
};

static inline BNRef add_bn(PlanBase& p, const std::string& name, int C) {
  BNRef r;
  r.g_off = add_tensor(p.params, p.param_numel, name + ".weight", {C});
  r.b_off = add_tensor(p.params, p.param_numel, name + ".bias", {C});
  r.rm_off = add_tensor(p.buffers, p.buffer_numel, name + ".running_mean", {C});
  r.rv_off = add_tensor(p.buffers, p.buffer_numel, name + ".running_var", {C});
  return r;
}

static inline size_t carve(size_t& cursor, size_t bytes) {
  size_t o = cursor;
  cursor = align_up(cursor + bytes, 256);
  return o;
}

#define PROF(cls_, flops_, bytes_, call_)                      \
  do {                                                        \
    p.prof.begin((cls_), st);                                 \
    rc = (call_);                                             \
    p.prof.end(st);                                           \
    if (p.prof.on) { p.prof.flops[(cls_)] += (flops_); p.prof.bytes[(cls_)] += (bytes_); } \
    if (rc) return rc;                                        \
  } while (0)

static inline double conv_flops(const ConvShape& s) {
  return 2.0 * s.N * s.OH() * s.OW() * (double)s.Cout * s.Cin * s.kh * s.kw;
}
static inline double conv_bytes(const ConvShape& s, size_t es, int extra_in_shaped = 0) {
  double in = (double)s.N * s.H * s.W * s.Cin, out = (double)s.N * s.OH() * s.OW() * s.Cout;
  return (in * (1 + extra_in_shaped) + out) * es + (double)s.Cout * s.Cin * s.kh * s.kw * es;
}

PlanBase* make_resnet_plan(int arch, int N, int H, int W, int dtype, int* rc);
PlanBase* make_densenet_plan(int N, int H, int W, int dtype, bool feature_map, int* rc);
PlanBase* make_vgg_plan(int N, int H, int W, int dtype, int* rc);
PlanBase* make_mobilenet_plan(int N, int H, int W, int dtype, int* rc);
PlanBase* make_efficientnet_plan(int variant, int N, int H, int W, int dtype, int* rc);
```

multimodal-model-skin-lesion-classifier_amd/csrc/wgrad.hip:

```cpp
#include <stdlib.h>

#include "conv.h"
#include "ops.h"

template <typename T> struct WG;
template <> struct WG<bf16_t> { static constexpr int MS = 32; };
template <> struct WG<float> { static constexpr int MS = 16; };

template <typename T, int PITCH> __device__ __forceinline__ int wg_swz(int row) {
  if constexpr (sizeof(T) == 4) {
    return (row & 1) << 2;
  } else if constexpr (PITCH % 256 == 0) {
    return ((row & 3) | (((row >> 3) & 1) << 2)) << 1;
  } else {
    return (((row >> 1) & 1) | (((row >> 3) & 1) << 1)) << 1;
  }
}

__device__ uint4 g_wzero_page[16];

__device__ __forceinline__ uint2 lds_read_tr16_b64(const unsigned char* p) {
  s16x4_t v = __builtin_amdgcn_ds_read_tr16_b64_v4i16(
      (__attribute__((address_space(3))) s16x4_t*)(p));
  return __builtin_bit_cast(uint2, v);
}

template <typename T, int BO, int BKK, int MS>
__device__ __forceinline__ void wg_compute(const unsigned char* Xb, const unsigned char* Yb,
                                           f32x4_t (&acc)[BKK / 32][BO / 32], int wo, int wk, int l15, int g) {
  constexpr int PX = BO * (int)sizeof(T), PY = BKK * (int)sizeof(T);
  constexpr int FO = BO / 32, FK = BKK / 32;
  if constexpr (sizeof(T) == 2) {
      const int q = l15 >> 2, pp = l15 & 3;
#pragma unroll
      for (int ks = 0; ks < MS / 32; ++ks) {
        uint4 fx[FO], fy[FK];
        const int r0 = 32 * ks + 8 * g + q, r1 = r0 + 4;
#pragma unroll
        for (int j = 0; j < FO; ++j) {
          int colb = (wo * (BO / 2) + j * 16 + 4 * pp) * 2;
          uint2 lo = lds_read_tr16_b64(Xb + r0 * PX + (((colb >> 4) ^ wg_swz<T, PX>(r0)) << 4) + (colb & 15));
          uint2 hi = lds_read_tr16_b64(Xb + r1 * PX + (((colb >> 4) ^ wg_swz<T, PX>(r1)) << 4) + (colb & 15));
          fx[j] = make_uint4(lo.x, lo.y, hi.x, hi.y);
        }
#pragma unroll
        for (int i = 0; i < FK; ++i) {
          int colb = (wk * (BKK / 2) + i * 16 + 4 * pp) * 2;
          uint2 lo = lds_read_tr16_b64(Yb + r0 * PY + (((colb >> 4) ^ wg_swz<T, PY>(r0)) << 4) + (colb & 15));
          uint2 hi = lds_read_tr16_b64(Yb + r1 * PY + (((colb >> 4) ^ wg_swz<T, PY>(r1)) << 4) + (colb & 15));
          fy[i] = make_uint4(lo.x, lo.y, hi.x, hi.y);
        }
#pragma unroll
        for (int i = 0; i < FK; ++i)
#pragma unroll
          for (int j = 0; j < FO; ++j)
            acc[i][j] = __builtin_amdgcn_mfma_f32_16x16x32_bf16(__builtin_bit_cast(bf16x8_t, fy[i]),
                                                                __builtin_bit_cast(bf16x8_t, fx[j]), acc[i][j], 0, 0, 0);
      }
    } else {
#pragma unroll
      for (int ks = 0; ks < MS / 4; ++ks) {
        const int row = 4 * ks + g;
        float fx[FO], fy[FK];
#pragma unroll
        for (int j = 0; j < FO; ++j) {
          int col = wo * (BO / 2) + j * 16 + l15;
          fx[j] = *reinterpret_cast<const float*>(Xb + row * PX + ((((col >> 2) ^ wg_swz<T, PX>(row)) << 4) | ((col & 3) << 2)));
        }
#pragma unroll
        for (int i = 0; i < FK; ++i) {
          int col = wk * (BKK / 2) + i * 16 + l15;
          fy[i] = *reinterpret_cast<const float*>(Yb + row * PY + ((((col >> 2) ^ wg_swz<T, PY>(row)) << 4) | ((col & 3) << 2)));
        }
#pragma unroll
        for (int i = 0; i < FK; ++i)
#pragma unroll
          for (int j = 0; j < FO; ++j)
            acc[i][j] = __builtin_amdgcn_mfma_f32_16x16x4f32(fy[i], fx[j], acc[i][j], 0, 0, 0);
      }
    }
}

template <typename T, int BO, int BKK, int MSF, int PF, bool S1 = false>
__global__ __launch_bounds__(256, 2) void wgrad_kernel(const WgradArgs p) {
  constexpr int EPC = DT<T>::EPC, MS = WG<T>::MS * MSF;
  constexpr int PX = BO * (int)sizeof(T), PY = BKK * (int)sizeof(T);
  constexpr int X_BYTES = MS * PX, Y_BYTES = MS * PY;
  constexpr int CPR_X = BO / EPC, CPR_Y = BKK / EPC;
  constexpr int NX = MS * CPR_X / 256 > 0 ? MS * CPR_X / 256 : 1;
  constexpr int NY = MS * CPR_Y / 256 > 0 ? MS * CPR_Y / 256 : 1;
  static_assert(MS * CPR_X % 256 == 0 && MS * CPR_Y % 256 == 0, "tile/thread mismatch");
  constexpr int FO = BO / 32, FK = BKK / 32;
  __shared__ __attribute__((aligned(16))) unsigned char smem[2 * (X_BYTES + Y_BYTES)];
  unsigned char* Xs = smem;
  unsigned char* Ys = smem + 2 * X_BYTES;

  const int tid = threadIdx.x;
  int tile = xcd_remap(blockIdx.x, gridDim.x);
  const int kb = tile % p.nblk_k; tile /= p.nblk_k;
  const int ob = tile % p.nblk_o;
  const int split = tile / p.nblk_o;
  const int o0 = ob * BO, k0 = kb * BKK;
  const int m_begin = split * p.m_per_split;
  const int m_end = min(p.M, m_begin + p.m_per_split);

  int x_row[NX], x_ch[NX];
#pragma unroll
  for (int i = 0; i < NX; ++i) { int idx = tid + 256 * i; x_row[i] = idx / CPR_X; x_ch[i] = idx - x_row[i] * CPR_X; }
  int y_row[NY], y_ch[NY], y_c[NY], y_oy[NY], y_ox[NY], y_img[NY], y_dy[NY], y_dx[NY];
  const int ohw = p.OH * p.OW;
#pragma unroll
  for (int i = 0; i < NY; ++i) {
    int idx = tid + 256 * i;
    y_row[i] = idx / CPR_Y; y_ch[i] = idx - y_row[i] * CPR_Y;
    int kidx = k0 + y_ch[i] * EPC;
    int tap = kidx / p.C;
    y_c[i] = kidx - tap * p.C;
    y_dy[i] = p.offy[tap]; y_dx[i] = p.offx[tap];
    int m = m_begin + y_row[i];
    int img = m / ohw, rem = m - img * ohw;
    y_img[i] = img; y_oy[i] = rem / p.OW; y_ox[i] = rem - y_oy[i] * p.OW;
  }
  const unsigned char* dy_b = reinterpret_cast<const unsigned char*>(p.dy);
  const unsigned char* in_b = reinterpret_cast<const unsigned char*>(p.in);

  static_assert(NX <= 4 && NY <= 4 && NX != 3 && NY != 3, "staging registers are written out for 1, 2 or 4 chunks per thread");
  const u32x4_t z4 = {0, 0, 0, 0};
  u32x4_t rxA0 = z4, rxA1 = z4, rxA2 = z4, rxA3 = z4, ryA0 = z4, ryA1 = z4, ryA2 = z4, ryA3 = z4;
#ifdef MMSKIN_ABLATE
  const int abl = p.ablate;
#else
  constexpr int abl = 0;
#endif
  int m_stage = m_begin;
  const unsigned char* zero_page = reinterpret_cast<const unsigned char*>(g_wzero_page);
  const int OWr = p.OW, OHr = p.OH;
  const int inv_ow = (65536 + OWr - 1) / OWr, inv_oh = (65536 + OHr - 1) / OHr;

#define LOAD_X(i, R)                                                                                   \
  {                                                                                                    \
    const int m = m_stage + x_row[i];                                                                  \
    const unsigned char* src = dy_b + ((size_t)m * p.Cout + o0 + x_ch[i] * EPC) * sizeof(T);           \
    R = *reinterpret_cast<const u32x4_t*>(m < m_end ? src : zero_page);                                \
  }
#define LOAD_Y(i, R)                                                                                   \
  { if constexpr (S1) {                                                                                \
    const int m = m_stage + y_row[i];                                                                  \
    const unsigned char* src = in_b + ((int64_t)m * p.Cpitch + y_c[i]) * (int)sizeof(T);               \
    R = *reinterpret_cast<const u32x4_t*>(m < m_end ? src : zero_page);                                \
  } else {                                                                                             \
    const int m = m_stage + y_row[i];                                                                  \
    const int iy = y_oy[i] * p.Sy + y_dy[i], ix = y_ox[i] * p.Sx + y_dx[i];                            \
    const bool ok = m < m_end && (unsigned)iy < (unsigned)p.IH && (unsigned)ix < (unsigned)p.IW;       \
    const unsigned char* src =                                                                         \
        in_b + ((int64_t)((y_img[i] * p.IH + iy) * p.IW + ix) * p.Cpitch + y_c[i]) * (int)sizeof(T);   \
    R = *reinterpret_cast<const u32x4_t*>(ok ? src : zero_page);                                       \
                                                    \
    int nx = y_ox[i] + MS;                                                                             \
    const int qy = (nx * inv_ow) >> 16;                                                                \
    nx -= qy * OWr;                                                                                    \
    const int ny = y_oy[i] + qy;                                                                       \
    const int qi = (ny * inv_oh) >> 16;                                                                \
    y_ox[i] = nx; y_oy[i] = ny - qi * OHr; y_img[i] += qi;                                             \
  } }
#define LOAD_STAGE(S)                                                                                  \
  do {                                                                                                 \
    if (!(abl & 1)) { LOAD_X(0, rx##S##0) if constexpr (NX > 1) LOAD_X(1 % NX, rx##S##1)               \
    if constexpr (NX > 2) { LOAD_X(2 % NX, rx##S##2) LOAD_X(3 % NX, rx##S##3) } }                      \
    if (!(abl & 2)) { LOAD_Y(0, ry##S##0) if constexpr (NY > 1) LOAD_Y(1 % NY, ry##S##1)               \
    if constexpr (NY > 2) { LOAD_Y(2 % NY, ry##S##2) LOAD_Y(3 % NY, ry##S##3) } }                      \
    m_stage += MS;                                                                                     \
  } while (0)
#define ST_X(buf, i, R) *reinterpret_cast<u32x4_t*>(Xs + (buf) * X_BYTES + x_row[i] * PX + ((x_ch[i] ^ wg_swz<T, PX>(x_row[i])) << 4)) = R;
#define ST_Y(buf, i, R) *reinterpret_cast<u32x4_t*>(Ys + (buf) * Y_BYTES + y_row[i] * PY + ((y_ch[i] ^ wg_swz<T, PY>(y_row[i])) << 4)) = R;
#define STORE_STAGE(buf, S)                                                                            \
  if (!(abl & 16)) do {                                                                                \
    ST_X(buf, 0, rx##S##0) if constexpr (NX > 1) ST_X(buf, 1 % NX, rx##S##1)                           \
    if constexpr (NX > 2) { ST_X(buf, 2 % NX, rx##S##2) ST_X(buf, 3 % NX, rx##S##3) }                  \
    ST_Y(buf, 0, ry##S##0) if constexpr (NY > 1) ST_Y(buf, 1 % NY, ry##S##1)                           \
    if constexpr (NY > 2) { ST_Y(buf, 2 % NY, ry##S##2) ST_Y(buf, 3 % NY, ry##S##3) }                  \
  } while (0)

  const int wid = tid >> 6, lane = tid & 63, l15 = lane & 15, g = lane >> 4;
  const int wo = wid >> 1, wk = wid & 1;
  f32x4_t acc[FK][FO];
#pragma unroll
  for (int i = 0; i < FK; ++i)
#pragma unroll
    for (int j = 0; j < FO; ++j) acc[i][j] = f32x4_t{0.f, 0.f, 0.f, 0.f};

  const int nstage = (m_end - m_begin + MS - 1) / MS;
  static_assert(PF == 1, "prefetch depth");
  if (nstage > 0) { LOAD_STAGE(A); STORE_STAGE(0, A); }
  __syncthreads();
  for (int s = 0; s < nstage; ++s) {
    const int cur = s & 1;
    if (s + 1 < nstage) LOAD_STAGE(A);
    if (!(abl & 4)) wg_compute<T, BO, BKK, MS>(Xs + cur * X_BYTES, Ys + cur * Y_BYTES, acc, wo, wk, l15, g);
    if (s + 1 < nstage) STORE_STAGE(cur ^ 1, A);
    __syncthreads();
  }

  float* slab = p.slab + (size_t)split * p.Cout * p.Ktot;
  if (abl & 8) return;
#pragma unroll
  for (int i = 0; i < FK; ++i)
#pragma unroll
    for (int j = 0; j < FO; ++j) {
      int cout = o0 + wo * (BO / 2) + j * 16 + l15;
      int kidx = k0 + wk * (BKK / 2) + i * 16 + g * 4;
      *reinterpret_cast<float4*>(slab + (size_t)cout * p.Ktot + kidx) =
          make_float4(acc[i][j][0], acc[i][j][1], acc[i][j][2], acc[i][j][3]);
    }
}

__global__ void wgrad_reduce_kernel(const float* __restrict__ slab, float* __restrict__ dw, int nsplit,
                                    int Cout, int C, int ntaps, int Coutv, int Cv) {
  const int Ktot = C * ntaps;
  const size_t total = (size_t)Cout * Ktot;
  for (size_t i = blockIdx.x * (size_t)blockDim.x + threadIdx.x; i < total; i += (size_t)gridDim.x * blockDim.x) {
    float s = 0.f;
    for (int k = 0; k < nsplit; ++k) s += slab[k * total + i];
    int cout = (int)(i / Ktot), kk = (int)(i - (size_t)cout * Ktot);
    int tap = kk / C, c = kk - tap * C;
    if (cout < Coutv && c < Cv) dw[((size_t)cout * Cv + c) * ntaps + tap] = s;
  }
}

__global__ __launch_bounds__(256) void wgrad_slab_group_kernel(const float4* __restrict__ slab, float4* __restrict__ part,
                                                               int nsplit, int total4, int per) {
  const int c = blockIdx.x * 256 + threadIdx.x;
  if (c >= total4) return;
  const int r0 = blockIdx.y * per, r1 = min(nsplit, r0 + per);
  float4 a0 = make_float4(0.f, 0.f, 0.f, 0.f), a1 = a0, a2 = a0, a3 = a0;
  const float4* src = slab + (size_t)r0 * total4 + c;
  int r = r0;
#define ACC4(a, u) a.x += u.x; a.y += u.y; a.z += u.z; a.w += u.w;
  for (; r + 3 < r1; r += 4, src += (size_t)4 * total4) {
    const float4 u0 = src[0], u1 = src[total4], u2 = src[(size_t)2 * total4], u3 = src[(size_t)3 * total4];
    ACC4(a0, u0) ACC4(a1, u1) ACC4(a2, u2) ACC4(a3, u3)
  }
  for (; r < r1; ++r, src += total4) { const float4 u = src[0]; ACC4(a0, u) }
  part[(size_t)blockIdx.y * total4 + c] =
      make_float4((a0.x + a1.x) + (a2.x + a3.x), (a0.y + a1.y) + (a2.y + a3.y), (a0.z + a1.z) + (a2.z + a3.z), (a0.w + a1.w) + (a2.w + a3.w));
}
__global__ __launch_bounds__(256) void wgrad_reduce4_kernel(const float4* __restrict__ slab, float* __restrict__ dw, int nsplit,
                                                            int Cout, int C, int ntaps, int Coutv, int Cv) {
  const int Ktot = C * ntaps;
  const int total4 = Cout * (Ktot / 4);
  const int i = blockIdx.x * 256 + threadIdx.x;
  if (i >= total4) return;
  float4 a0 = make_float4(0.f, 0.f, 0.f, 0.f), a1 = a0;
  const float4* src = slab + i;
  int k = 0;
  for (; k + 1 < nsplit; k += 2, src += (size_t)2 * total4) { const float4 u0 = src[0], u1 = src[total4]; ACC4(a0, u0) ACC4(a1, u1) }
  if (k < nsplit) { const float4 u = src[0]; ACC4(a0, u) }
#undef ACC4
  const float v[4] = {a0.x + a1.x, a0.y + a1.y, a0.z + a1.z, a0.w + a1.w};
  const int e = i * 4;
  const int cout = e / Ktot, kk = e - cout * Ktot;
  const int tap = kk / C, c = kk - tap * C;
  if (cout >= Coutv) return;
#pragma unroll
  for (int j = 0; j < 4; ++j)
    if (c + j < Cv) dw[((size_t)cout * Cv + c + j) * ntaps + tap] = v[j];
}

__global__ __launch_bounds__(256) void wgrad_reduce4_lanes_kernel(const float4* __restrict__ slab, float* __restrict__ dw, int nsplit,
                                                                  int Cout, int C, int ntaps, int Coutv, int Cv) {
  __shared__ float4 red[4][64];
  const int Ktot = C * ntaps;
  const int total4 = Cout * (Ktot / 4);
  const int cx = threadIdx.x & 63, ry = threadIdx.x >> 6;
  const int i = blockIdx.x * 64 + cx;
  float4 a0 = make_float4(0.f, 0.f, 0.f, 0.f), a1 = a0, a2 = a0, a3 = a0;
#define ACC4(a, u) a.x += u.x; a.y += u.y; a.z += u.z; a.w += u.w;
  if (i < total4) {
    const float4* src = slab + (size_t)ry * total4 + i;
    int k = ry;
    for (; k + 12 < nsplit; k += 16, src += (size_t)16 * total4) {
      const float4 u0 = src[0], u1 = src[(size_t)4 * total4], u2 = src[(size_t)8 * total4], u3 = src[(size_t)12 * total4];
      ACC4(a0, u0) ACC4(a1, u1) ACC4(a2, u2) ACC4(a3, u3)
    }
    for (; k < nsplit; k += 4, src += (size_t)4 * total4) { const float4 u = src[0]; ACC4(a0, u) }
  }
  red[ry][cx] = make_float4((a0.x + a1.x) + (a2.x + a3.x), (a0.y + a1.y) + (a2.y + a3.y), (a0.z + a1.z) + (a2.z + a3.z), (a0.w + a1.w) + (a2.w + a3.w));
  __syncthreads();
  if (ry != 0 || i >= total4) return;
  float4 t = red[0][cx];
  ACC4(t, red[1][cx]) ACC4(t, red[2][cx]) ACC4(t, red[3][cx])
#undef ACC4
  const float v[4] = {t.x, t.y, t.z, t.w};
  const int e = i * 4;
  const int cout = e / Ktot, kk = e - cout * Ktot;
  const int tap = kk / C, c = kk - tap * C;
  if (cout >= Coutv) return;
#pragma unroll
  for (int j = 0; j < 4; ++j)
    if (c + j < Cv) dw[((size_t)cout * Cv + c + j) * ntaps + tap] = v[j];
}

static void wgrad_plan(int M, int Cout, int Ktot, int MS, int& BO, int& BKK, int& nsplit, int& mps, int ntaps = 1) {
  BO = (Cout % 128 == 0) ? 128 : 64;
  BKK = (Ktot % 128 == 0) ? 128 : 64;
  MS *= (BO + BKK == 128) ? 4 : 2;
  int tiles = (Cout / BO) * (Ktot / BKK);
  constexpr int one_round = 512, two_rounds = 1024;
  const int target = (ntaps == 1 || tiles >= 64) ? one_round : two_rounds;
  int want = target / tiles > 0 ? target / tiles : 1;
  int max_split = M / (MS * 4) > 0 ? M / (MS * 4) : 1;
  nsplit = want < max_split ? want : max_split;
  if (nsplit < 1) nsplit = 1;
  mps = ceil_div(ceil_div(M, nsplit), MS) * MS;
  nsplit = ceil_div(M, mps);
}

#define WG_DIRECT_SPLITS 32
#define WG_GROUPS 64

static int reduce_slabs(float* slab, int nsplit, int Cout, int Ktot, float* dw, int C_for_layout, int ntaps_for_layout,
                        int cout_valid, int cin_valid, hipStream_t st) {
  size_t total = (size_t)Cout * Ktot;
  const int total4 = (int)(total / 4);
  const float* src = slab;
  int nsrc = nsplit;
  if (nsplit > WG_DIRECT_SPLITS && C_for_layout % 4 == 0) {
    const int coutv = cout_valid > 0 ? cout_valid : Cout, cv = cin_valid > 0 ? cin_valid : C_for_layout;
    hipLaunchKernelGGL(wgrad_reduce4_lanes_kernel, dim3(ceil_div(total4, 64)), dim3(256), 0, st, reinterpret_cast<const float4*>(slab),
                       dw, nsplit, Cout, C_for_layout, ntaps_for_layout, coutv, cv);
    HIP_CHECK_RET(hipGetLastError());
    return MMSKIN_OK;
  }
  if (nsplit > WG_DIRECT_SPLITS) {
    float* slab2 = slab + (size_t)nsplit * total;
    int G = ceil_div(262144, total4);
    const int g_lo = ceil_div(nsplit, 32), g_hi = nsplit / 2 < WG_GROUPS ? nsplit / 2 : WG_GROUPS;
    if (G < g_lo) G = g_lo;
    if (G > g_hi) G = g_hi;
    const int per = ceil_div(nsplit, G);
    G = ceil_div(nsplit, per);
    hipLaunchKernelGGL(wgrad_slab_group_kernel, dim3(ceil_div(total4, 256), G), dim3(256), 0, st,
                       reinterpret_cast<const float4*>(slab), reinterpret_cast<float4*>(slab2), nsplit, total4, per);
    HIP_CHECK_RET(hipGetLastError());
    src = slab2;
    nsrc = G;
  }
  const int coutv = cout_valid > 0 ? cout_valid : Cout, cv = cin_valid > 0 ? cin_valid : C_for_layout;
  if (C_for_layout % 4 == 0) {
    hipLaunchKernelGGL(wgrad_reduce4_kernel, dim3(ceil_div(total4, 256)), dim3(256), 0, st, reinterpret_cast<const float4*>(src),
                       dw, nsrc, Cout, C_for_layout, ntaps_for_layout, coutv, cv);
  } else {
    int blocks = (int)((total + 255) / 256);
    if (blocks > 65536) blocks = 65536;
    hipLaunchKernelGGL(wgrad_reduce_kernel, dim3(blocks), dim3(256), 0, st, src, dw, nsrc, Cout, C_for_layout,
                       ntaps_for_layout, coutv, cv);
  }
  HIP_CHECK_RET(hipGetLastError());
  return MMSKIN_OK;
}

template <typename T>
static size_t slab_bytes(int M, int Cout, int Ktot, int ntaps) {
  int BO, BKK, ns, mps;
  wgrad_plan(M, Cout, Ktot, WG<T>::MS, BO, BKK, ns, mps, ntaps);
  if constexpr (sizeof(T) == 2) {
    WgradRingPlan rp;
    for (int simple = 0; simple < 2; ++simple)
      if (wgrad_ring_tile(M, Cout, Ktot, rp, simple != 0) && rp.nsplit > ns) ns = rp.nsplit;
  }
  return (size_t)(ns + (ns > WG_DIRECT_SPLITS ? WG_GROUPS : 0)) * Cout * Ktot * sizeof(float);
}
static size_t wgrad3_slab_bytes(const ConvShape& s);
size_t conv_wgrad_slab_bytes(const ConvShape& s) {
  int M = s.N * s.OH() * s.OW(), K = s.kh * s.kw * s.Cin;
  size_t a = slab_bytes<float>(M, s.Cout, K, s.kh * s.kw), b = slab_bytes<bf16_t>(M, s.Cout, K, s.kh * s.kw);
  const size_t c = wgrad3_slab_bytes(s);
  if (c > b) b = c;
  return a > b ? a : b;
}
size_t stem_wgrad_slab_bytes(int N, int OH, int OW) {
  size_t a = slab_bytes<float>(N * OH * OW, 64, 256, 8), b = slab_bytes<bf16_t>(N * OH * OW, 64, 256, 8);
  return a > b ? a : b;
}

template <typename T, int BO, int BKK, int MSF>
static int launch_wg(WgradArgs& a, hipStream_t st) {
  a.nblk_o = a.Cout / BO;
  a.nblk_k = a.Ktot / BKK;
  int grid = a.nblk_o * a.nblk_k * a.nsplit;
  if (a.simple1x1 && sizeof(T) == 2 && BO >= 64 && BKK >= 64 && BO + BKK >= 192) hipLaunchKernelGGL((wgrad_kernel<T, BO, BKK, MSF, 1, true>), dim3(grid), dim3(256), 0, st, a);
  else hipLaunchKernelGGL((wgrad_kernel<T, BO, BKK, MSF, 1>), dim3(grid), dim3(256), 0, st, a);
  HIP_CHECK_RET(hipGetLastError());
  return MMSKIN_OK;
}


template <typename T>
static int run_wgrad(WgradArgs& a, float* dw, int C_for_layout, int ntaps_for_layout, hipStream_t st,
                     int cout_valid = 0, int cin_valid = 0) {
  ARG_CHECK(a.Cout % 64 == 0 && a.Ktot % 64 == 0, "wgrad: Cout=%d Ktot=%d must be multiples of 64", a.Cout, a.Ktot);
  ARG_CHECK(a.C % DT<T>::EPC == 0, "wgrad: C=%d", a.C);
  ARG_CHECK(a.OW <= 240 && a.OH <= 240, "wgrad: output %dx%d too large for the 16-bit reciprocal pixel stepping", a.OH, a.OW);
  if constexpr (sizeof(T) == 2) {
    WgradRingPlan rp;
    if (wgrad_ring_plan(a, rp)) {
      int rc = wgrad_ring_launch(a, rp, st);
      if (rc) return rc;
      return reduce_slabs(a.slab, a.nsplit, a.Cout, a.Ktot, dw, C_for_layout, ntaps_for_layout, cout_valid, cin_valid, st);
    }
  }
  int BO, BKK;
  wgrad_plan(a.M, a.Cout, a.Ktot, WG<T>::MS, BO, BKK, a.nsplit, a.m_per_split, a.ntaps);
  a.ablate = 0;
#ifdef MMSKIN_ABLATE
  { const char* v = getenv("MMSKIN_WGRAD_ABLATE"); a.ablate = v ? atoi(v) : 0; }
#endif
  int rc;
  if (BO == 128 && BKK == 128) rc = launch_wg<T, 128, 128, 2>(a, st);
  else if (BO == 128) rc = launch_wg<T, 128, 64, 2>(a, st);
  else if (BKK == 128) rc = launch_wg<T, 64, 128, 2>(a, st);
  else rc = launch_wg<T, 64, 64, 4>(a, st);
  if (rc) return rc;
  return reduce_slabs(a.slab, a.nsplit, a.Cout, a.Ktot, dw, C_for_layout, ntaps_for_layout, cout_valid, cin_valid, st);
}


struct Wgrad3Args {
  const bf16_t* dy; const bf16_t* in; float* slab;
  int N, H, W, C, Cout;
  int R, spi;
  int total_stages, stages_per_split, nsplit;
  int nblk_o, nblk_c;
  int yrows;
};
#define W3_PITCH 144
#define W3_XROWS 64
#define W3_YROWS 176
#define W3_LDS_BYTES (2 * (W3_XROWS + W3_YROWS) * W3_PITCH)

__global__ __launch_bounds__(256, 2) void wgrad3x3_kernel(const Wgrad3Args p) {
  extern __shared__ __attribute__((aligned(16))) unsigned char smem3[];
  unsigned char* Xs = smem3;
  unsigned char* Ys = smem3 + 2 * W3_XROWS * W3_PITCH;
  constexpr int X_BYTES = W3_XROWS * W3_PITCH, Y_BYTES = W3_YROWS * W3_PITCH;
  const int tid = threadIdx.x;
  int tile = xcd_remap(blockIdx.x, gridDim.x);
  const int cb = tile % p.nblk_c; tile /= p.nblk_c;
  const int ob = tile % p.nblk_o;
  const int split = tile / p.nblk_o;
  const int o0 = ob * 64, c0 = cb * 64;
  const int W = p.W, H = p.H, W2 = W + 2, R = p.R;
  const int st_begin = split * p.stages_per_split;
  const int st_end = min(p.total_stages, st_begin + p.stages_per_split);
  int img = st_begin / p.spi, y0 = (st_begin - img * p.spi) * R;

  const int ch = tid & 7;
  int x_r[2], x_pix[2];
  bool x_ok[2];
#pragma unroll
  for (int i = 0; i < 2; ++i) {
    const int slot = (tid >> 3) + 32 * i;
    x_r[i] = slot / W;
    x_pix[i] = slot;
    x_ok[i] = slot < R * W;
  }
  int y_wr[6], y_pix[6];
  bool y_ok[6];
#pragma unroll
  for (int i = 0; i < 6; ++i) {
    const int j = (tid >> 3) + 32 * i;
    const int wr = j / W2, wc = j - wr * W2;
    y_wr[i] = wr - 1;
    y_pix[i] = (wr - 1) * W + (wc - 1);
    y_ok[i] = j < p.yrows && wc >= 1 && wc <= W;
  }
  const u32x4_t z4 = {0, 0, 0, 0};
  u32x4_t rx0 = z4, rx1 = z4, ry0 = z4, ry1 = z4, ry2 = z4, ry3 = z4, ry4 = z4, ry5 = z4;
#define W3_LOADX(i, Rg)                                                                                         \
  {                                                                                                             \
    const bool ok = x_ok[i] && (y0 + x_r[i] < H);                                                               \
    const bf16_t* src = p.dy + ((size_t)((img * H + y0) * W + x_pix[i]) * p.Cout + o0 + ch * 8);                \
    Rg = z4;                                                                                                    \
    if (ok) Rg = *reinterpret_cast<const u32x4_t*>(src);                                                        \
  }
#define W3_LOADY(i, Rg)                                                                                         \
  {                                                                                                             \
    const bool ok = y_ok[i] && (unsigned)(y0 + y_wr[i]) < (unsigned)H;                                          \
    const bf16_t* src = p.in + ((int64_t)((img * H + y0) * W + y_pix[i]) * p.C + c0 + ch * 8);                  \
    Rg = z4;                                                                                                    \
    if (ok) Rg = *reinterpret_cast<const u32x4_t*>(src);                                                        \
  }
#define W3_LOAD_STAGE()                                                                                         \
  do {                                                                                                          \
    W3_LOADX(0, rx0) W3_LOADX(1, rx1)                                                                           \
    W3_LOADY(0, ry0) W3_LOADY(1, ry1) W3_LOADY(2, ry2) W3_LOADY(3, ry3) W3_LOADY(4, ry4) W3_LOADY(5, ry5)       \
  } while (0)
#define W3_STX(buf, i, Rg) *reinterpret_cast<u32x4_t*>(Xs + (buf) * X_BYTES + ((tid >> 3) + 32 * i) * W3_PITCH + ch * 16) = Rg;
#define W3_STY(buf, i, Rg)                                                                                      \
  if ((tid >> 3) + 32 * i < W3_YROWS) *reinterpret_cast<u32x4_t*>(Ys + (buf) * Y_BYTES + ((tid >> 3) + 32 * i) * W3_PITCH + ch * 16) = Rg;
#define W3_STORE_STAGE(buf)                                                                                     \
  do {                                                                                                          \
    W3_STX(buf, 0, rx0) W3_STX(buf, 1, rx1)                                                                     \
    W3_STY(buf, 0, ry0) W3_STY(buf, 1, ry1) W3_STY(buf, 2, ry2) W3_STY(buf, 3, ry3) W3_STY(buf, 4, ry4) W3_STY(buf, 5, ry5) \
  } while (0)
#define W3_ADVANCE()                                                                                            \
  do { y0 += R; if (y0 >= H) { y0 = 0; ++img; } } while (0)

  const int wid = tid >> 6, lane = tid & 63, l15 = lane & 15, g = lane >> 4;
  const int q = l15 >> 2, pp = l15 & 3;
  const int wo = wid >> 1, wk = wid & 1;
  int xa[2][2], ya[2][2];
#pragma unroll
  for (int ks = 0; ks < 2; ++ks)
#pragma unroll
    for (int h = 0; h < 2; ++h) {
      const int k = 32 * ks + 8 * g + q + 4 * h;
      xa[ks][h] = k * W3_PITCH + (wo * 32 + 4 * pp) * 2;
      const int r = k / W, x = k - r * W;
      const int brow = k < R * W ? r * W2 + x : 0;
      ya[ks][h] = brow * W3_PITCH + (wk * 32 + 4 * pp) * 2;
    }
  f32x4_t acc[9][2][2];
#pragma unroll
  for (int t = 0; t < 9; ++t)
#pragma unroll
    for (int i = 0; i < 2; ++i)
#pragma unroll
      for (int j = 0; j < 2; ++j) acc[t][i][j] = f32x4_t{0.f, 0.f, 0.f, 0.f};

#define W3_COMPUTE(buf)                                                                                         \
  do {                                                                                                          \
    const unsigned char* Xb = Xs + (buf) * X_BYTES;                                                             \
    const unsigned char* Yb = Ys + (buf) * Y_BYTES;                                                             \
    _Pragma("unroll") for (int ks = 0; ks < 2; ++ks) {                                                          \
      uint4 fx[2];                                                                                              \
      _Pragma("unroll") for (int j = 0; j < 2; ++j) {                                                           \
        uint2 lo = lds_read_tr16_b64(Xb + xa[ks][0] + j * 32);                                                  \
        uint2 hi = lds_read_tr16_b64(Xb + xa[ks][1] + j * 32);                                                  \
        fx[j] = make_uint4(lo.x, lo.y, hi.x, hi.y);                                                             \
      }                                                                                                         \
      _Pragma("unroll") for (int t = 0; t < 9; ++t) {                                                           \
        const int tb = ((t / 3) * W2 + (t % 3)) * W3_PITCH;                                                     \
        _Pragma("unroll") for (int i = 0; i < 2; ++i) {                                                         \
          uint2 lo = lds_read_tr16_b64(Yb + ya[ks][0] + tb + i * 32);                                           \
          uint2 hi = lds_read_tr16_b64(Yb + ya[ks][1] + tb + i * 32);                                           \
          const uint4 fy = make_uint4(lo.x, lo.y, hi.x, hi.y);                                                  \
          _Pragma("unroll") for (int j = 0; j < 2; ++j)                                                         \
            acc[t][i][j] = __builtin_amdgcn_mfma_f32_16x16x32_bf16(__builtin_bit_cast(bf16x8_t, fy),            \
                                                                   __builtin_bit_cast(bf16x8_t, fx[j]), acc[t][i][j], 0, 0, 0); \
        }                                                                                                       \
      }                                                                                                         \
    }                                                                                                           \
  } while (0)

  if (st_begin < st_end) { W3_LOAD_STAGE(); W3_STORE_STAGE(0); }
  __syncthreads();
  for (int s = st_begin; s < st_end; ++s) {
    const int cur = (s - st_begin) & 1;
    if (s + 1 < st_end) { W3_ADVANCE(); W3_LOAD_STAGE(); }
    W3_COMPUTE(cur);
    if (s + 1 < st_end) W3_STORE_STAGE(cur ^ 1);
    __syncthreads();
  }

  const int Ktot = 9 * p.C;
  float* slab = p.slab + (size_t)split * p.Cout * Ktot;
#pragma unroll
  for (int t = 0; t < 9; ++t)
#pragma unroll
    for (int i = 0; i < 2; ++i)
#pragma unroll
      for (int j = 0; j < 2; ++j) {
        const int cout = o0 + wo * 32 + j * 16 + l15;
        const int kidx = t * p.C + c0 + wk * 32 + i * 16 + g * 4;
        *reinterpret_cast<float4*>(slab + (size_t)cout * Ktot + kidx) =
            make_float4(acc[t][i][j][0], acc[t][i][j][1], acc[t][i][j][2], acc[t][i][j][3]);
      }
}

static bool wgrad3_plan(const ConvShape& s, Wgrad3Args& a) {
  if (s.kh != 3 || s.kw != 3 || s.stride != 1 || s.pad != 1) return false;
  if (s.Cin % 64 || s.Cout % 64 || s.W > 64 || s.W < 1) return false;
  int R = 64 / s.W;
  if (R > s.H) R = s.H;
  if ((R + 2) * (s.W + 2) > W3_YROWS) return false;
  a.N = s.N; a.H = s.H; a.W = s.W; a.C = s.Cin; a.Cout = s.Cout;
  a.R = R; a.spi = ceil_div(s.H, R);
  a.total_stages = s.N * a.spi;
  a.nblk_o = s.Cout / 64; a.nblk_c = s.Cin / 64;
  a.yrows = (R + 2) * (s.W + 2);
  const int tiles = a.nblk_o * a.nblk_c;
  static const int target = env_knob("MMSKIN_WGRAD3_BLOCKS", 512);
  int ns = target / tiles > 0 ? target / tiles : 1;
  constexpr int min_stages = 16;
  if (ns > a.total_stages / min_stages) ns = a.total_stages / min_stages > 0 ? a.total_stages / min_stages : 1;
  if (ns > a.total_stages) ns = a.total_stages;
  a.stages_per_split = ceil_div(a.total_stages, ns);
  a.nsplit = ceil_div(a.total_stages, a.stages_per_split);
  return true;
}
static size_t wgrad3_slab_bytes(const ConvShape& s) {
  Wgrad3Args a = {};
  int ns = wgrad3_plan(s, a) ? a.nsplit : 0, nr = 0;
  if (wgrad3_ring_takes(s, &nr) && nr > ns) ns = nr;
  if (!ns) return 0;
  return (size_t)(ns + (ns > WG_DIRECT_SPLITS ? WG_GROUPS : 0)) * s.Cout * 9 * s.Cin * sizeof(float);
}
static int launch_wgrad3(const ConvShape& s, Wgrad3Args& a, const bf16_t* dout, const bf16_t* in, float* slab, float* dw,
                         hipStream_t st, int cout_valid, int cin_valid) {
  a.dy = dout; a.in = in; a.slab = slab;
  HIP_CHECK_RET(opt_in_dynamic_lds(reinterpret_cast<const void*>(wgrad3x3_kernel), W3_LDS_BYTES));
  hipLaunchKernelGGL(wgrad3x3_kernel, dim3(a.nblk_o * a.nblk_c * a.nsplit), dim3(256), W3_LDS_BYTES, st, a);
  HIP_CHECK_RET(hipGetLastError());
  return reduce_slabs(slab, a.nsplit, s.Cout, 9 * s.Cin, dw, s.Cin, 9, cout_valid, cin_valid, st);
}

template <typename T>
int launch_conv_wgrad(const ConvShape& s, const T* dout, const T* in, float* slab, float* dw_oihw,
                      hipStream_t st, int cout_valid, int cin_valid) {
  ARG_CHECK(s.kh * s.kw <= MMSKIN_MAX_TAPS, "wgrad: too many taps");
  if constexpr (sizeof(T) == 2) {
    int nsr = 0;
    if (wgrad3_ring_takes(s, &nsr)) {
      int rc = launch_wgrad3_ring(s, dout, in, slab, st, &nsr);
      if (rc) return rc;
      return reduce_slabs(slab, nsr, s.Cout, 9 * s.Cin, dw_oihw, s.Cin, 9, cout_valid, cin_valid, st);
    }
    Wgrad3Args a3 = {};
    if (wgrad3_plan(s, a3)) return launch_wgrad3(s, a3, dout, in, slab, dw_oihw, st, cout_valid, cin_valid);
  }
  WgradArgs a = {};
  a.dy = dout; a.in = in; a.slab = slab;
  a.N = s.N; a.IH = s.H; a.IW = s.W; a.C = s.Cin; a.Cpitch = s.Cin;
  a.OH = s.OH(); a.OW = s.OW();
  a.Cout = s.Cout; a.Ktot = s.kh * s.kw * s.Cin;
  a.Sy = s.stride; a.Sx = s.stride; a.ntaps = s.kh * s.kw;
  a.M = s.N * a.OH * a.OW;
  a.simple1x1 = (s.kh == 1 && s.kw == 1 && s.stride == 1 && s.pad == 0) ? 1 : 0;
  for (int r = 0; r < s.kh; ++r)
    for (int q = 0; q < s.kw; ++q) {
      a.offy[r * s.kw + q] = (int8_t)(r - s.pad);
      a.offx[r * s.kw + q] = (int8_t)(q - s.pad);
    }
  return run_wgrad<T>(a, dw_oihw, s.Cin, s.kh * s.kw, st, cout_valid, cin_valid);
}

template <typename T>
int launch_stem_conv_wgrad(int N, int OH, int OW, int Hp, int Wp, const T* dout, const T* img4,
                           float* slab, float* dwv, hipStream_t st) {
  WgradArgs a = {};
  a.dy = dout; a.in = img4; a.slab = slab;
  a.N = N; a.IH = Hp; a.IW = Wp / 2; a.C = 32; a.Cpitch = 8;
  a.OH = OH; a.OW = OW; a.Cout = 64; a.Ktot = 256;
  a.Sy = 2; a.Sx = 1; a.ntaps = 8;
  a.M = N * OH * OW;
  for (int r = 0; r < 8; ++r) { a.offy[r] = (int8_t)r; a.offx[r] = 0; }
  return run_wgrad<T>(a, dwv, 256, 1, st);
}

size_t vgg_first_wgrad_slab_bytes(int N, int H, int W) {
  size_t a = slab_bytes<float>(N * H * W, 64, 128, 4), b = slab_bytes<bf16_t>(N * H * W, 64, 128, 4);
  return a > b ? a : b;
}
template <typename T>
int launch_vgg_first_conv_wgrad(int N, int H, int W, int Hp, int Wp, const T* dout, const T* img8, float* slab,
                                float* dwv, hipStream_t st, int stride) {
  const int OH = (H + 2 - 3) / stride + 1, OW = (W + 2 - 3) / stride + 1;
  WgradArgs a = {};
  a.dy = dout; a.in = img8; a.slab = slab;
  a.N = N; a.IH = Hp; a.IW = Wp; a.C = 32; a.Cpitch = 8;
  a.OH = OH; a.OW = OW; a.Cout = 64; a.Ktot = 128;
  a.Sy = stride; a.Sx = stride; a.ntaps = 4;
  a.M = N * OH * OW;
  for (int r = 0; r < 4; ++r) { a.offy[r] = (int8_t)(r < 3 ? r : 0); a.offx[r] = 0; }
  return run_wgrad<T>(a, dwv, 128, 1, st);
}

#define INST(T)                                                                                   \
  template int launch_vgg_first_conv_wgrad<T>(int, int, int, int, int, const T*, const T*, float*, float*, hipStream_t, int); \
  template int launch_conv_wgrad<T>(const ConvShape&, const T*, const T*, float*, float*, hipStream_t, int, int); \
  template int launch_stem_conv_wgrad<T>(int, int, int, int, int, const T*, const T*, float*, float*, hipStream_t);
INST(float)
INST(bf16_t)
```

multimodal-model-skin-lesion-classifier_amd/mmskin/_lib.py:

```python
import ctypes
import os
import re

_HERE = os.path.dirname(os.path.abspath(__file__))
LIB_PATH = os.path.join(os.path.dirname(_HERE), "libmmskin_hip.so")
HEADER_PATH = os.path.join(os.path.dirname(os.path.dirname(_HERE)), "include", "mmskin.h")

F32, BF16 = 0, 1
LINEAR_SMALL, LINEAR_BIG_F32, LINEAR_BIG_BF16, LINEAR_PADDED_BF16 = 0, 1, 2, 3

_lib = None

c_f = ctypes.c_void_p
_i, _i64, _f = ctypes.c_int, ctypes.c_int64, ctypes.c_float
_u64 = ctypes.c_uint64
_P = ctypes.c_void_p

_SIGNATURES = {
    "mmskin_last_error": (ctypes.c_char_p, []),
    "mmskin_version": (_i, []),
    "mmskin_backbone_create": (_i, [ctypes.c_char_p, _i, _i, _i, _i, ctypes.POINTER(_P)]),
    "mmskin_backbone_destroy": (None, [_P]),
    "mmskin_backbone_num_tensors": (_i, [_P, _i]),
    "mmskin_backbone_tensor_info": (_i, [_P, _i, _i, ctypes.c_char_p, _i, ctypes.POINTER(_i64),
                                         ctypes.POINTER(_i64), ctypes.POINTER(_i), ctypes.POINTER(_i64)]),
    "mmskin_backbone_param_numel": (_i64, [_P]),
    "mmskin_backbone_buffer_numel": (_i64, [_P]),
    "mmskin_backbone_workspace_bytes": (_i64, [_P]),
    "mmskin_backbone_feature_dim": (_i, [_P]),
    "mmskin_backbone_feature_hw": (_i, [_P, _P, _P]),
    "mmskin_backbone_set_option": (_i, [_P, ctypes.c_char_p, _i]),
    "mmskin_backbone_set_pointer": (_i, [_P, ctypes.c_char_p, _P]),
    "mmskin_backbone_num_grad_segments": (_i, [_P, ctypes.POINTER(ctypes.c_int)]),
    "mmskin_backbone_grad_segment": (_i, [_P, _i, ctypes.POINTER(ctypes.c_int64), ctypes.POINTER(ctypes.c_int64)]),
    "mmskin_backbone_wait_grad_segment": (_i, [_P, _i, _P]),
    "mmskin_backbone_last_conv_shape": (_i, [_P, _P, _P, _P]),
    "mmskin_backbone_last_conv_export": (_i, [_P, _P, _P, _P]),
    "mmskin_backbone_last_conv_grad": (_i, [_P, _P, _P, _P, _P]),
    "mmskin_mdnet_fuse_forward": (_i, [_P] * 5 + [_i64, _i, _P]),
    "mmskin_mdnet_fuse_backward": (_i, [_P] * 9 + [_i64, _i, _P]),
    "mmskin_backbone_profile_enable": (_i, [_P, _i]),
    "mmskin_backbone_profile_read": (_i, [_P, ctypes.POINTER(ctypes.c_double), ctypes.POINTER(ctypes.c_double),
                                          ctypes.POINTER(ctypes.c_double), ctypes.POINTER(_i64)]),
    "mmskin_backbone_num_units": (_i, [_P]),
    "mmskin_backbone_unit_info": (_i, [_P, _i, ctypes.c_char_p, _i, ctypes.POINTER(_i64)]),
    "mmskin_backbone_forward": (_i, [_P, _P, _P, _P, _P, _P, _i, _P]),
    "mmskin_backbone_forward_u8": (_i, [_P, _P, _P, _P, _P, _P, _P, _i, _P]),
    "mmskin_backbone_backward": (_i, [_P, _P, _P, _P, _P, _P]),
    "mmskin_conv2d_workspace_bytes": (_i64, [_i] * 9),
    "mmskin_conv2d_forward": (_i, [_P, _P, _P] + [_i] * 10 + [_P, _P]),
    "mmskin_conv2d_time": (ctypes.c_double, [_i] * 11 + [_P, _P]),
    "mmskin_conv2d_wgrad_time": (ctypes.c_double, [_i] * 11 + [_P, _P]),
    "mmskin_conv2d_dgrad_time": (ctypes.c_double, [_i] * 11 + [_P, _P]),
    "mmskin_conv2d_backward": (_i, [_P] * 5 + [_i] * 10 + [_P, _P]),
    "mmskin_conv_pipe_launches": (_i64, []),
    "mmskin_wgrad_ring_launches": (_i64, []),
    "mmskin_conv3x3_c64_launches": (_i64, []),
    "mmskin_stem7x7_launches": (_i64, []),
    "mmskin_conv2d_dgrad_fused_rows": (_i, [_i] * 9),
    "mmskin_conv2d_dgrad_fused": (_i, [_P] * 8 + [_i] * 9 + [_P, _P]),
    "mmskin_wgrad3_ring_launches": (_i64, []),
    "mmskin_abn_workspace_bytes": (_i64, [_i] * 5),
    "mmskin_abn_backward": (_i, [_P] * 6 + [_i] * 5 + [_P, _P, _P, _P]),
    "mmskin_adam_step": (_i, [_P] * 4 + [_i64] + [ctypes.c_double] * 5 + [_i64, _P]),
    "mmskin_abn_backward_kept_gram": (_i, [_P] * 6 + [_i] * 5 + [_P, _P, _P, _P]),
    "mmskin_conv1x1_gram_stats": (_i, [_P, _P] + [_i] * 5 + [_P, _P, _P, _P]),
    "mmskin_batchnorm_workspace_bytes": (_i64, [_i] * 4),
    "mmskin_batchnorm_forward": (_i, [_P] * 8 + [_i] * 4 + [_f, _f, _i, _i, _P, _P]),
    "mmskin_batchnorm_backward": (_i, [_P] * 9 + [_i] * 6 + [_P, _P]),
    "mmskin_stem_workspace_bytes": (_i64, [_i] * 3),
    "mmskin_stem_forward": (_i, [_P] * 5 + [_i] * 3 + [_f, _i, _P, _P]),
    "mmskin_stem_backward": (_i, [_P] * 8 + [_i] * 3 + [_f, _i, _P, _P]),
    "mmskin_linear_forward": (_i, [_P] * 4 + [_i] * 4 + [_P]),
    "mmskin_linear_backward": (_i, [_P] * 8 + [_i] * 3 + [_P]),
    "mmskin_linear_gelu_backward": (_i, [_P] * 8 + [_i] * 3 + [_P]),
    "mmskin_linear_x16_pitch": (_i, [_i, _i, _i]),
    "mmskin_linear_route": (_i, [_i, _i, _i]),
    "mmskin_linear_forward_keep": (_i, [_P] * 6 + [_i] * 4 + [_P]),
    "mmskin_linear_backward_keep": (_i, [_P] * 9 + [_i] * 3 + [_P]),
    "mmskin_gelu_forward_bf16": (_i, [_P, _P, _i64, _i, _i, _P]),
    "mmskin_linear_forward_x16": (_i, [_P] * 5 + [_i] * 4 + [_P]),
    "mmskin_layernorm_forward": (_i, [_P] * 6 + [_i, _i, _f, _i, _P]),
    "mmskin_layernorm_backward": (_i, [_P] * 9 + [_i, _i, _i, _P]),
    "mmskin_sigmoid_gate_forward": (_i, [_P] * 3 + [_i64, _P]),
    "mmskin_sigmoid_gate_backward": (_i, [_P] * 5 + [_i64, _P]),
    "mmskin_gated_mix_forward": (_i, [_P] * 4 + [_i64, _P]),
    "mmskin_gated_mix_backward": (_i, [_P] * 7 + [_i64, _P]),
    "mmskin_metablock_gate_forward": (_i, [_P] * 4 + [_i64, _P]),
    "mmskin_metablock_gate_backward": (_i, [_P] * 7 + [_i64, _P]),
    "mmskin_dropout_forward": (_i, [_P] * 3 + [_i64, _f, _u64, _u64, _P]),
    "mmskin_attn_dropout_forward": (_i, [_P] * 3 + [_i64, _i, _f, _u64, _u64, _P]),
    "mmskin_dropout_backward": (_i, [_P] * 3 + [_i64, _f, _P]),
    "mmskin_concat2_forward": (_i, [_P] * 3 + [_i] * 3 + [_P]),
    "mmskin_concat2_backward": (_i, [_P] * 3 + [_i] * 3 + [_P]),
    "mmskin_attention_forward": (_i, [_P] * 5 + [_i] * 4 + [_f, _u64, _u64, _P]),
    "mmskin_attention_backward": (_i, [_P] * 8 + [_i] * 4 + [_f, _u64, _u64, _P]),
    "mmskin_bmm": (_i, [_P] * 3 + [_i] * 4 + [_i64] * 8 + [_P]),
    "mmskin_softmax_forward": (_i, [_P] * 4 + [_i64, _i, _i64, _f, _i, _P]),
    "mmskin_gelu_tanh_forward": (_i, [_P, _P, _i64, _P]),
    "mmskin_gelu_tanh_backward": (_i, [_P, _P, _P, _i64, _P]),
    "mmskin_colsum": (_i, [_P, _P, _i, _i, _P]),
    "mmskin_dwconv3_scratch_floats": (_i64, [_i, _i, _i, _i]),
    "mmskin_dwconv3_forward": (_i, [_P] * 4 + [_i] * 4 + [_P]),
    "mmskin_dwconv3_backward": (_i, [_P] * 7 + [_i] * 4 + [_P]),
    "mmskin_conv_pos_enc_forward": (_i, [_P] * 5 + [_i] * 4 + [_P]),
    "mmskin_conv_pos_enc_backward": (_i, [_P] * 8 + [_i] * 4 + [_P]),
    "mmskin_factor_attention_scratch_floats": (_i64, [_i] * 5),
    "mmskin_factor_attention_forward": (_i, [_P] * 11 + [_i] * 4 + [_P]),
    "mmskin_factor_attention_backward": (_i, [_P] * 18 + [_i] * 4 + [_P]),
    "mmskin_conv_pos_enc_tokens_scratch_floats": (_i64, [_i] * 4),
    "mmskin_conv_pos_enc_tokens_forward": (_i, [_P] * 4 + [_i] * 4 + [_P]),
    "mmskin_conv_pos_enc_tokens_backward": (_i, [_P] * 7 + [_i] * 4 + [_P]),
    "mmskin_scale_add_forward": (_i, [_P] * 4 + [_i64, _i, _P]),
    "mmskin_scale_mul": (_i, [_P] * 3 + [_i64, _i, _i, _P]),
    "mmskin_token_mean_forward": (_i, [_P, _P, _i, _i, _i, _i, _P]),
    "mmskin_token_mean_backward": (_i, [_P, _P, _i, _i, _i, _i, _P]),
    "mmskin_softmax_backward": (_i, [_P] * 3 + [_i64, _i, _f, _P]),
    "mmskin_add": (_i, [_P, _P, _P, _i64, _i64, _P]),
    "mmskin_gelu_forward": (_i, [_P, _P, _i64, _P]),
    "mmskin_gelu_backward": (_i, [_P, _P, _P, _i64, _P]),
    "mmskin_embedding_forward": (_i, [_P] * 3 + [_i] * 4 + [_P]),
    "mmskin_embedding_backward": (_i, [_P] * 3 + [_i] * 4 + [_P]),
    "mmskin_direct_conv2d_forward": (_i, [_P] * 4 + [_i] * 10 + [_P]),
    "mmskin_direct_conv2d_backward": (_i, [_P] * 5 + [_i] * 9 + [_P]),
    "mmskin_linear_forward_ex": (_i, [_P, _i, _P, _P, _P, _i, _i, _i, _i, _i, _P]),
    "mmskin_attention_rows_forward": (_i, [_P] * 5 + [_i] * 4 + [_P, _P, _f, _f, _u64, _u64, _P]),
    "mmskin_attention_rows_backward": (_i, [_P] * 9 + [_i] * 4 + [_P, _P, _f, _f, _u64, _u64, _P]),
    "mmskin_window_attention_forward": (_i, [_P] * 5 + [_i] * 6 + [_i64] * 4 + [_f, _f, _u64, _u64, _P]),
    "mmskin_window_attention_backward": (_i, [_P] * 9 + [_i] * 6 + [_i64] * 4 + [_f, _f, _u64, _u64, _P]),
    "mmskin_channel_attention_scratch_floats": (_i64, [_i, _i, _i]),
    "mmskin_channel_attention_forward": (_i, [_P] * 6 + [_i] * 4 + [_i64] * 4 + [_f, _P]),
    "mmskin_channel_attention_backward": (_i, [_P] * 9 + [_i] * 4 + [_i64] * 4 + [_f, _P]),
    "mmskin_linear_lane": (_i, [_P, _i, _P, _i, _P, _P, _P, _f, _u64, _u64, _P, _i, _i, _i, _i, _i, _P]),
    "mmskin_layernorm_forward_mixed": (_i, [_P] * 5 + [_i, _i, _f, _P]),
    "mmskin_flash_attention_forward": (_i, [_P] * 7 + [_i] * 4 + [_P, _i, _f, _i, _f, _u64, _u64, _P]),
    "mmskin_flash_attention_backward": (_i, [_P] * 14 + [_i] * 4 + [_P, _f, _i, _f, _u64, _u64, _P]),
    "mmskin_set_linear_dtype": (_i, [_i]),
    "mmskin_get_linear_dtype": (_i, []),
    "mmskin_im2col_forward": (_i, [_P] + [_i] * 8 + [_P, _P]),
    "mmskin_im2col_backward": (_i, [_P] + [_i] * 8 + [_P, _P]),
    "mmskin_resize_u8": (_i, [_P, _i, _i, _i, _P, _i, _i, _P]),
    "mmskin_metadata_encode": (_i, [_P, _i, _P, _i, _P, _i, _P, _P, _f, _P, _i, _P]),
    "mmskin_pool_gap_forward": (_i, [_P] * 3 + [_i] * 5 + [_P]),
    "mmskin_pool_gap_backward": (_i, [_P] * 3 + [_i] * 5 + [_P]),
    "mmskin_star_relu_forward_bf16": (_i, [_P] * 4 + [_i64, _i, _i, _P]),
    "mmskin_linear_star_relu_backward_keep": (_i, [_P] * 9 + [_i] * 3 + [_P]),
    "mmskin_star_relu_forward": (_i, [_P] * 4 + [_i64, _P]),
    "mmskin_star_relu_backward": (_i, [_P] * 5 + [_i64, _P]),
    "mmskin_dw7_star_scratch_floats": (_i64, [_i] * 4),
    "mmskin_dw7_star_forward": (_i, [_P] * 5 + [_i] * 4 + [_P]),
    "mmskin_dw7_star_backward": (_i, [_P] * 9 + [_i] * 4 + [_P]),
}


class MMSkinError(RuntimeError):
    pass


def declared_symbols():
    with open(HEADER_PATH) as f:
        text = f.read()
    return sorted(set(re.findall(r"\b(mmskin_[a-z0-9_]+)\s*\(", text)))


def load():
    global _lib
    if _lib is not None:
        return _lib
    if not os.path.exists(LIB_PATH):
        raise MMSkinError(
            f"{LIB_PATH} not found: build it with `python __graft_entry__.py` (or `make -C "
            f"{os.path.join(os.path.dirname(_HERE), 'csrc')}`).  There is no CPU fallback.")
    lib = ctypes.CDLL(LIB_PATH)
    for name, (res, args) in _SIGNATURES.items():
        fn = getattr(lib, name)
        fn.restype = res
        fn.argtypes = args
    _lib = lib
    return lib


def check(rc):
    if rc != 0:
        msg = load().mmskin_last_error()
        raise MMSkinError(f"mmskin error {rc}: {msg.decode() if msg else ''}")


def ptr(t):
    return None if t is None else ctypes.c_void_p(t.data_ptr())


_raw_stream = None


def stream():
    global _raw_stream
    if _raw_stream is None:
        import torch
        get, dev = getattr(torch._C, "_cuda_getCurrentRawStream", None), getattr(torch._C, "_cuda_getDevice", None)
        if get is not None and dev is not None:
            _raw_stream = lambda: get(dev())
        else:
            _raw_stream = lambda: torch.cuda.current_stream().cuda_stream
    return ctypes.c_void_p(_raw_stream())


_fns = {}


def call(name, *args):
    fn = _fns.get(name)
    if fn is None:
        fn = _fns[name] = getattr(load(), name)
    rc = fn(*args)
    if rc != 0:
        check(rc)
```

Before: 15190 images/sec.

## Batch per-layer wgrad split-K slab reductions into one grouped kernel per block

```diff
diff --git a/include/mmskin.h b/include/mmskin.h
--- a/include/mmskin.h
+++ b/include/mmskin.h
@@ -64,6 +64,8 @@
 int64_t mmskin_conv_pipe_launches(void);
 int64_t mmskin_wgrad_ring_launches(void);
 int64_t mmskin_wgrad3_ring_launches(void);
+int mmskin_wgrad_reduce_group(const float* slabs, int64_t slab_numel, float* dw, int64_t dw_numel, int n, const int64_t* desc,
+                              int layerwise, void* stream);
 int64_t mmskin_abn_workspace_bytes(int N, int Cw, int C4, int H, int W);
 int mmskin_abn_backward(const float* g, const float* y, const float* w, const float* cA, const float* cB, const float* cC, int N, int Cw,
                         int C4, int H, int W, float* dy, float* dw, void* workspace, void* stream);
diff --git a/multimodal-model-skin-lesion-classifier_amd/csrc/backbone.hip b/multimodal-model-skin-lesion-classifier_amd/csrc/backbone.hip
--- a/multimodal-model-skin-lesion-classifier_amd/csrc/backbone.hip
+++ b/multimodal-model-skin-lesion-classifier_amd/csrc/backbone.hip
@@ -15,6 +15,7 @@
   size_t gram_off = 0;
   bool fwd2p = false;
   size_t abn_coef_off = 0;
+  int wg_entry = -1;
   size_t rows() const { return (size_t)s.N * s.OH() * s.OW(); }
 };
 
@@ -25,7 +26,10 @@
   size_t in_off;
   int in_C, in_H, in_W;
   int seg_done = -1;
+  int wg_flush = -1;
 };
+
+struct WgGroup { int first, count, nblocks; };
 
 struct Plan : PlanBase {
   int arch;
@@ -39,6 +43,18 @@
   size_t off_abn_wd2 = 0, off_abn_bias2 = 0;
   size_t off_abn_sgx = 0, off_abn_slab2 = 0, off_abn_S2 = 0, off_abn_cs2 = 0;
   size_t maxact_bytes = 0, stat_bytes = 0;
+  size_t off_gslab = 0;
+  std::vector<WgradGroupEntry> wg_tab;
+  std::vector<WgGroup> wg_groups;
+  int wg_final = -1;
+  WgradGroupEntry* wg_tab_dev = nullptr;
+  int ensure_wg_table() {
+    if (wg_tab_dev) return MMSKIN_OK;
+    HIP_CHECK_RET(hipMalloc((void**)&wg_tab_dev, wg_tab.size() * sizeof(WgradGroupEntry)));
+    HIP_CHECK_RET(hipMemcpy(wg_tab_dev, wg_tab.data(), wg_tab.size() * sizeof(WgradGroupEntry), hipMemcpyHostToDevice));
+    return MMSKIN_OK;
+  }
+  ~Plan() override { if (wg_tab_dev) (void)hipFree(wg_tab_dev); }
 
   int forward(const void* image, const float* norm6, const float* params, float* buffers, unsigned char* ws,
               float* features, bool training, hipStream_t st) override;
@@ -144,7 +160,7 @@
   p.off_img4 = carve(cur, (size_t)p.N * p.Hp * p.Wp * 4 * es);
   p.off_wf = carve(cur, (size_t)wf * es);
   p.off_wd = carve(cur, (size_t)wd * es);
-  size_t stat_rows_max = 0, maxact = 0, slab_max = stem_wgrad_slab_bytes(p.N, p.OH0, p.OW0), partial_max = 0;
+  size_t stat_rows_max = 0, maxact = 0, slab_max = 0, partial_max = 0;
   int maxC = 64;
   for (Unit& u : p.units) {
     size_t rows = u.rows();
@@ -152,7 +168,6 @@
     if (sr > stat_rows_max) stat_rows_max = sr;
     if (rows * u.s.Cout > maxact) maxact = rows * u.s.Cout;
     if ((size_t)u.s.N * u.s.H * u.s.W * u.s.Cin > maxact && !u.stem) maxact = (size_t)u.s.N * u.s.H * u.s.W * u.s.Cin;
-    if (!u.stem) { size_t sb = conv_wgrad_slab_bytes(u.s); if (sb > slab_max) slab_max = sb; }
     size_t pr = (size_t)bn_bwd_partial_rows(rows, u.s.Cout) * 2 * u.s.Cout * sizeof(float);
     if (pr > partial_max) partial_max = pr;
     pr = ((rows + 127) / 128 + 4) * 2 * u.s.Cout * sizeof(float);
@@ -250,6 +265,45 @@
   p.off_dwv = carve(cur, 64 * 256 * sizeof(float));
   p.off_red = carve(cur, bn_reduce_scratch_bytes(maxC));
   p.off_red_b = carve(cur, bn_reduce_scratch_bytes(maxC));
+  {
+    const int nb = (int)p.blocks.size();
+    size_t gcur = 0, gmax = 0;
+    WgGroup grp = {0, 0, 0};
+    int rc = MMSKIN_OK;
+    auto add = [&](Unit& u) {
+      if (rc) return;
+      WgradSlabs d = {};
+      if (u.stem) rc = p.dtype == 1 ? stem_wgrad_describe<bf16_t>(p.N, p.OH0, p.OW0, p.Hp, p.Wp, &d) : stem_wgrad_describe<float>(p.N, p.OH0, p.OW0, p.Hp, p.Wp, &d);
+      else rc = p.dtype == 1 ? conv_wgrad_describe<bf16_t>(u.s, &d) : conv_wgrad_describe<float>(u.s, &d);
+      if (rc) return;
+      u.wg_entry = (int)p.wg_tab.size();
+      rc = wgrad_group_add(p.wg_tab, d, (long long)(gcur / sizeof(float)), u.stem ? (long long)(p.off_dwv / sizeof(float)) : (long long)u.w_off,
+                           u.stem ? 1 : 0, &grp.nblocks);
+      gcur = align_up(gcur + (size_t)d.nsplit * d.Cout * d.Ktot * sizeof(float), 256);
+      ++grp.count;
+    };
+    auto close = [&]() {
+      p.wg_groups.push_back(grp);
+      if (gcur > gmax) gmax = gcur;
+      gcur = 0;
+      grp = WgGroup{(int)p.wg_tab.size(), 0, 0};
+      return (int)p.wg_groups.size() - 1;
+    };
+    for (int bi = nb - 1; bi >= 0; --bi) {
+      Block& b = p.blocks[bi];
+      const bool alg = p.dtype == 1 && bi + 1 < nb;
+      for (int i = (int)b.units.size() - 1; i >= 0; --i) {
+        Unit& u = p.units[b.units[i]];
+        if (!(alg && u.abn && i + 1 == (int)b.units.size())) add(u);
+      }
+      if (b.ds >= 0 && !(alg && p.units[b.ds].abn)) add(p.units[b.ds]);
+      if (bi > 0) b.wg_flush = close();
+    }
+    add(p.units[0]);
+    p.wg_final = close();
+    if (rc) return rc;
+    p.off_gslab = carve(cur, gmax);
+  }
   p.ws_bytes = cur;
   return MMSKIN_OK;
 }
@@ -308,6 +362,7 @@
   float* stat_sq = reinterpret_cast<float*>(ws + p.off_stat + p.stat_bytes);
   int rc;
   if ((rc = p.ensure_table())) return rc;
+  if (training && (rc = p.ensure_wg_table())) return rc;
   const bool folded_eval = !training && !p.keep_raw_eval;
   const bool reuse = folded_eval && p.reuse_staged && p.staged_eval_ws == ws;
   p.staged_eval_ws = folded_eval ? ws : nullptr;
@@ -439,11 +494,13 @@
                   hipStream_t st) {
   T* wd = reinterpret_cast<T*>(ws + p.off_wd);
   float* slab = reinterpret_cast<float*>(ws + p.off_slab);
+  float* gslab = reinterpret_cast<float*>(ws + p.off_gslab);
   float* partial = reinterpret_cast<float*>(ws + p.off_partial);
   float* cA = reinterpret_cast<float*>(ws + p.off_coefbwd);
   T* S[7];
   for (int i = 0; i < 7; ++i) S[i] = reinterpret_cast<T*>(ws + p.off_scratch[i]);
   int rc;
+  if ((rc = p.ensure_wg_table())) return rc;
 
   auto bn_backward = [&](Unit& u, const T* dy, const T* ymask, int mode, T* dx, T* dz) -> int {
     const int C = u.s.Cout;
@@ -498,9 +555,13 @@
       HIP_CHECK_RET(hipStreamWaitEvent(p.side.s, p.side.ready[i], 0));
       ws_st = p.side.s;
     }
+    if (u.wg_entry < 0) { mmskin_set_error("backbone backward: unit without a weight-gradient slab"); return MMSKIN_ERR_ARG; }
+    const WgradGroupEntry& e = p.wg_tab[u.wg_entry];
+    WgradSlabs d = {};
     p.prof.begin(K_WGRAD, st);
-    int r = launch_conv_wgrad<T>(u.s, DX[i], uin, slab, grads + u.w_off, ws_st);
+    int r = launch_conv_wgrad<T>(u.s, DX[i], uin, gslab + e.slab_off, grads + u.w_off, ws_st, 0, 0, p.wgrad_layerwise ? nullptr : &d);
     p.prof.end(st);
+    if (!r && !p.wgrad_layerwise && d.nsplit != e.nsplit) { mmskin_set_error("backbone backward: split count differs from the plan's"); r = MMSKIN_ERR_ARG; }
     if (p.prof.on) { p.prof.flops[K_WGRAD] += conv_flops(u.s); p.prof.bytes[K_WGRAD] += conv_bytes(u.s, sizeof(T)); }
     if (r) return r;
     if (use_side) {
@@ -508,6 +569,15 @@
       p.side.done_valid[i] = true;
     }
     return MMSKIN_OK;
+  };
+  auto wgrad_flush = [&](int gi) -> int {
+    if (gi < 0 || p.wgrad_layerwise) return MMSKIN_OK;
+    const WgGroup& gr = p.wg_groups[gi];
+    p.prof.begin(K_WGRAD, st);
+    int r = launch_wgrad_reduce_group(p.wg_tab_dev + gr.first, gr.count, gr.nblocks, gslab, grads, reinterpret_cast<float*>(ws),
+                                      use_side ? p.side.s : st);
+    p.prof.end(st);
+    return r;
   };
   int dxi = 0;
   for (int i = 0; i < 2; ++i) p.side.g_done_valid[i] = false;
@@ -669,6 +739,7 @@
       }
     }
     T* t = g; g = gin; gin = t;
+    if ((rc = wgrad_flush(b.wg_flush))) return rc;
     if (b.seg_done >= 0 && (rc = p.segment_done(b.seg_done, st, use_side))) return rc;
   }
 
@@ -697,10 +768,13 @@
     wst = p.side.s;
   }
   p.prof.begin(K_WGRAD, st);
-  rc = launch_stem_conv_wgrad<T>(p.N, p.OH0, p.OW0, p.Hp, p.Wp, dx0, reinterpret_cast<const T*>(ws + p.off_img4), slab, dwv, wst);
+  WgradSlabs d0 = {};
+  rc = launch_stem_conv_wgrad<T>(p.N, p.OH0, p.OW0, p.Hp, p.Wp, dx0, reinterpret_cast<const T*>(ws + p.off_img4),
+                                 gslab + p.wg_tab[u0.wg_entry].slab_off, dwv, wst, p.wgrad_layerwise ? nullptr : &d0);
   p.prof.end(st);
   if (p.prof.on) p.prof.flops[K_WGRAD] += conv_flops(u0.s);
   if (rc) return rc;
+  if ((rc = wgrad_flush(p.wg_final))) return rc;
   if ((rc = stem_wgrad_unpack(dwv, grads + u0.w_off, wst))) return rc;
   if (use_side) {
     HIP_CHECK_RET(hipEventRecord(p.side.done[0], p.side.s));
@@ -870,6 +944,7 @@
   ARG_CHECK(h && key, "backbone_set_option: null argument");
   if (!strcmp(key, "keep_raw_eval")) { h->plan->keep_raw_eval = value != 0; return MMSKIN_OK; }
   if (!strcmp(key, "reuse_staged")) { h->plan->reuse_staged = value != 0; return MMSKIN_OK; }
+  if (!strcmp(key, "wgrad_layerwise")) { h->plan->wgrad_layerwise = value != 0; return MMSKIN_OK; }
   mmskin_set_error("backbone_set_option: unknown option '%s'", key);
   return MMSKIN_ERR_ARG;
 }
diff --git a/multimodal-model-skin-lesion-classifier_amd/csrc/conv.h b/multimodal-model-skin-lesion-classifier_amd/csrc/conv.h
--- a/multimodal-model-skin-lesion-classifier_amd/csrc/conv.h
+++ b/multimodal-model-skin-lesion-classifier_amd/csrc/conv.h
@@ -1,4 +1,6 @@
 #pragma once
+#include <vector>
+
 #include "common.h"
 
 struct ConvShape {
@@ -156,13 +158,33 @@
 int launch_conv3x3_c64_dgrad(const ConvShape& s, const bf16_t* dout, const bf16_t* wt_staged, bf16_t* din, DgradFuse* fuse, hipStream_t st);
 
 size_t conv_wgrad_slab_bytes(const ConvShape& s);
+struct WgradSlabs {
+  float* slab;
+  float* dw;
+  int nsplit, Cout, Ktot;
+  int C, ntaps;
+  int cout_valid, cin_valid;
+};
 template <typename T>
 int launch_conv_wgrad(const ConvShape& s, const T* dout, const T* in, float* slab, float* dw,
-                      hipStream_t st, int cout_valid = 0, int cin_valid = 0);
+                      hipStream_t st, int cout_valid = 0, int cin_valid = 0, WgradSlabs* defer = nullptr);
 size_t stem_wgrad_slab_bytes(int N, int OH, int OW);
 template <typename T>
 int launch_stem_conv_wgrad(int N, int OH, int OW, int Hp, int Wp, const T* dout, const T* img4,
-                           float* slab, float* dwv, hipStream_t st);
+                           float* slab, float* dwv, hipStream_t st, WgradSlabs* defer = nullptr);
+template <typename T> int conv_wgrad_describe(const ConvShape& s, WgradSlabs* out);
+template <typename T> int stem_wgrad_describe(int N, int OH, int OW, int Hp, int Wp, WgradSlabs* out);
+
+struct WgradGroupEntry {
+  long long slab_off, dw_off;
+  int dw_base;
+  int nsplit, Cout, C, ntaps, coutv, cv;
+  int blk0;
+  int cols;
+};
+int wgrad_group_add(std::vector<WgradGroupEntry>& tab, const WgradSlabs& d, long long slab_off, long long dw_off, int dw_base, int* nblocks);
+int launch_wgrad_reduce_group(const WgradGroupEntry* tab_dev, int nent, int nblocks, const float* slab_base, float* dw_base0, float* dw_base1,
+                              hipStream_t st);
 
 bool wgrad3_ring_takes(const ConvShape& s, int* nsplit);
 int launch_wgrad3_ring(const ConvShape& s, const bf16_t* dout, const bf16_t* in, float* slab, hipStream_t st, int* nsplit);
diff --git a/multimodal-model-skin-lesion-classifier_amd/csrc/plan.h b/multimodal-model-skin-lesion-classifier_amd/csrc/plan.h
--- a/multimodal-model-skin-lesion-classifier_amd/csrc/plan.h
+++ b/multimodal-model-skin-lesion-classifier_amd/csrc/plan.h
@@ -117,6 +117,7 @@
   virtual int backward(const float* dfeat, const float* params, unsigned char* ws, float* grads, hipStream_t st) = 0;
   bool keep_raw_eval = false;
   bool reuse_staged = false;
+  bool wgrad_layerwise = false;
   const void* staged_eval_ws = nullptr;
   virtual int last_conv_shape(int*, int*, int*) const { return MMSKIN_ERR_UNSUPPORTED; }
   virtual int last_conv_export(const unsigned char*, float*, hipStream_t) { return MMSKIN_ERR_UNSUPPORTED; }
diff --git a/multimodal-model-skin-lesion-classifier_amd/csrc/wgrad.hip b/multimodal-model-skin-lesion-classifier_amd/csrc/wgrad.hip
--- a/multimodal-model-skin-lesion-classifier_amd/csrc/wgrad.hip
+++ b/multimodal-model-skin-lesion-classifier_amd/csrc/wgrad.hip
@@ -359,6 +359,174 @@
   return MMSKIN_OK;
 }
 
+static int finish_slabs(float* slab, int nsplit, int Cout, int Ktot, float* dw, int C_for_layout, int ntaps_for_layout,
+                        int cout_valid, int cin_valid, hipStream_t st, WgradSlabs* defer, bool dry) {
+  if (defer) {
+    *defer = WgradSlabs{slab, dw, nsplit, Cout, Ktot, C_for_layout, ntaps_for_layout, cout_valid, cin_valid};
+    return MMSKIN_OK;
+  }
+  if (dry) return MMSKIN_OK;
+  return reduce_slabs(slab, nsplit, Cout, Ktot, dw, C_for_layout, ntaps_for_layout, cout_valid, cin_valid, st);
+}
+
+#define WGG_TILE_FLOATS 4736
+
+__global__ __launch_bounds__(256) void wgrad_reduce_group_kernel(const WgradGroupEntry* __restrict__ tab, int nent,
+                                                                 const float* __restrict__ slab_base, float* dw0, float* dw1) {
+  __shared__ float4 red[2][4][64];
+  __shared__ __attribute__((aligned(16))) float tile[WGG_TILE_FLOATS];
+  int lo = 0, hi = nent - 1;
+  while (lo < hi) {
+    const int mid = (lo + hi + 1) >> 1;
+    if (tab[mid].blk0 <= (int)blockIdx.x) lo = mid; else hi = mid - 1;
+  }
+  const WgradGroupEntry e = tab[lo];
+  const int K4 = e.C * e.ntaps / 4, total4 = e.Cout * K4;
+  const float4* slab = reinterpret_cast<const float4*>(slab_base + e.slab_off);
+  float* dw = (e.dw_base ? dw1 : dw0) + e.dw_off;
+  const int col0 = ((int)blockIdx.x - e.blk0) * e.cols;
+  const int ncols = min(e.cols, total4 - col0);
+  const bool lanes = e.nsplit > WG_DIRECT_SPLITS;
+  const int step = lanes ? 64 : 256;
+  const int cx = lanes ? (threadIdx.x & 63) : threadIdx.x, ry = lanes ? (threadIdx.x >> 6) : 0;
+  const int pitch = e.C + 4;
+  const int nsplit = e.nsplit;
+#define ACC4(a, u) a.x += u.x; a.y += u.y; a.z += u.z; a.w += u.w;
+  for (int base = 0, it = 0; base < ncols; base += step, ++it) {
+    const int j = base + cx;
+    const bool live = j < ncols;
+    const int i = col0 + j;
+    float4 v = make_float4(0.f, 0.f, 0.f, 0.f);
+    if (!lanes) {
+      if (live) {
+        float4 a0 = v, a1 = v;
+        const float4* src = slab + i;
+        int k = 0;
+        for (; k + 1 < nsplit; k += 2, src += (size_t)2 * total4) { const float4 u0 = src[0], u1 = src[total4]; ACC4(a0, u0) ACC4(a1, u1) }
+        if (k < nsplit) { const float4 u = src[0]; ACC4(a0, u) }
+        v = make_float4(a0.x + a1.x, a0.y + a1.y, a0.z + a1.z, a0.w + a1.w);
+      }
+    } else {
+      float4 a0 = v, a1 = v, a2 = v, a3 = v;
+      if (live) {
+        const float4* src = slab + (size_t)ry * total4 + i;
+        int k = ry;
+        for (; k + 12 < nsplit; k += 16, src += (size_t)16 * total4) {
+          const float4 u0 = src[0], u1 = src[(size_t)4 * total4], u2 = src[(size_t)8 * total4], u3 = src[(size_t)12 * total4];
+          ACC4(a0, u0) ACC4(a1, u1) ACC4(a2, u2) ACC4(a3, u3)
+        }
+        for (; k < nsplit; k += 4, src += (size_t)4 * total4) { const float4 u = src[0]; ACC4(a0, u) }
+      }
+      float4 (*rd)[64] = red[it & 1];
+      rd[ry][cx] = make_float4((a0.x + a1.x) + (a2.x + a3.x), (a0.y + a1.y) + (a2.y + a3.y), (a0.z + a1.z) + (a2.z + a3.z), (a0.w + a1.w) + (a2.w + a3.w));
+      __syncthreads();
+      if (ry == 0) {
+        v = rd[0][cx];
+        ACC4(v, rd[1][cx]) ACC4(v, rd[2][cx]) ACC4(v, rd[3][cx])
+      }
+    }
+    if (ry != 0 || !live) continue;
+    if (e.ntaps == 1) {
+      const int el = i * 4;
+      const int cout = el / e.C, c = el - cout * e.C;
+      if (cout >= e.coutv) continue;
+      float* dst = dw + (size_t)cout * e.cv + c;
+      if (c + 3 < e.cv && (reinterpret_cast<uintptr_t>(dst) & 15) == 0) {
+        *reinterpret_cast<float4*>(dst) = v;
+      } else {
+        const float vv[4] = {v.x, v.y, v.z, v.w};
+#pragma unroll
+        for (int q = 0; q < 4; ++q)
+          if (c + q < e.cv) dst[q] = vv[q];
+      }
+    } else {
+      const int r = j / K4, kk = (j - r * K4) * 4;
+      const int tap = kk / e.C, c = kk - tap * e.C;
+      *reinterpret_cast<float4*>(tile + (r * e.ntaps + tap) * pitch + c) = v;
+    }
+  }
+#undef ACC4
+  if (e.ntaps == 1) return;
+  __syncthreads();
+  const int row0 = col0 / K4, rowlen = e.cv * e.ntaps;
+  int nrows = ncols / K4;
+  if (row0 + nrows > e.coutv) nrows = e.coutv - row0;
+  float* out = dw + (size_t)row0 * rowlen;
+  for (int o = threadIdx.x; o < nrows * rowlen; o += 256) {
+    const int r = o / rowlen, q = o - r * rowlen;
+    const int c = q / e.ntaps, tap = q - c * e.ntaps;
+    out[o] = tile[(r * e.ntaps + tap) * pitch + c];
+  }
+}
+
+int wgrad_group_add(std::vector<WgradGroupEntry>& tab, const WgradSlabs& d, long long slab_off, long long dw_off, int dw_base, int* nblocks) {
+  ARG_CHECK(d.nsplit >= 1 && d.Cout >= 1 && d.C >= 4 && d.C % 4 == 0 && d.ntaps >= 1 && d.Ktot == d.C * d.ntaps,
+            "wgrad_group_add: nsplit=%d Cout=%d Ktot=%d C=%d ntaps=%d (C must be a multiple of 4, Ktot = C * ntaps)", d.nsplit, d.Cout, d.Ktot, d.C, d.ntaps);
+  ARG_CHECK(slab_off % 4 == 0 && (dw_base == 0 || dw_base == 1), "wgrad_group_add: slab offset %lld must be a multiple of 4 floats", slab_off);
+  ARG_CHECK((long long)d.Cout * d.Ktot < (1ll << 31), "wgrad_group_add: Cout=%d x Ktot=%d too large", d.Cout, d.Ktot);
+  WgradGroupEntry e = {};
+  e.slab_off = slab_off; e.dw_off = dw_off; e.dw_base = dw_base;
+  e.nsplit = d.nsplit; e.Cout = d.Cout; e.C = d.C; e.ntaps = d.ntaps;
+  e.coutv = d.cout_valid > 0 ? d.cout_valid : d.Cout;
+  e.cv = d.cin_valid > 0 ? d.cin_valid : d.C;
+  ARG_CHECK(e.coutv <= d.Cout && e.cv <= d.C, "wgrad_group_add: cout_valid=%d cin_valid=%d", d.cout_valid, d.cin_valid);
+  const int step = d.nsplit > WG_DIRECT_SPLITS ? 64 : 256, K4 = d.Ktot / 4;
+  if (d.ntaps == 1) {
+    e.cols = step;
+  } else {
+    int rows = step / K4 > 0 ? step / K4 : 1;
+    ARG_CHECK(rows * d.ntaps * (d.C + 4) <= WGG_TILE_FLOATS, "wgrad_group_add: a %d-tap row of %d channels does not fit the transposition tile", d.ntaps, d.C);
+    e.cols = rows * K4;
+  }
+  e.blk0 = *nblocks;
+  *nblocks += ceil_div(d.Cout * K4, e.cols);
+  tab.push_back(e);
+  return MMSKIN_OK;
+}
+
+int launch_wgrad_reduce_group(const WgradGroupEntry* tab_dev, int nent, int nblocks, const float* slab_base, float* dw_base0, float* dw_base1,
+                              hipStream_t st) {
+  ARG_CHECK(tab_dev && nent > 0 && nblocks > 0 && slab_base && dw_base0, "wgrad_reduce_group: empty group");
+  hipLaunchKernelGGL(wgrad_reduce_group_kernel, dim3(nblocks), dim3(256), 0, st, tab_dev, nent, slab_base, dw_base0, dw_base1);
+  HIP_CHECK_RET(hipGetLastError());
+  return MMSKIN_OK;
+}
+
+extern "C" int mmskin_wgrad_reduce_group(const float* slabs, int64_t slab_numel, float* dw, int64_t dw_numel, int n, const int64_t* desc,
+                                         int layerwise, void* stream) {
+  ARG_CHECK(slabs && dw && desc && n > 0, "wgrad_reduce_group: null argument");
+  hipStream_t st = (hipStream_t)stream;
+  std::vector<WgradGroupEntry> tab;
+  std::vector<WgradSlabs> ds;
+  int nblocks = 0;
+  for (int i = 0; i < n; ++i) {
+    const int64_t* q = desc + 9 * i;
+    WgradSlabs d = {const_cast<float*>(slabs) + q[0], dw + q[8], (int)q[1], (int)q[2], (int)q[3], (int)q[4], (int)q[5], (int)q[6], (int)q[7]};
+    ARG_CHECK(q[0] >= 0 && q[8] >= 0 && q[1] >= 1 && q[2] >= 1 && q[3] >= 4, "wgrad_reduce_group: entry %d", i);
+    int rc = wgrad_group_add(tab, d, q[0], q[8], 0, &nblocks);
+    if (rc) return rc;
+    const WgradGroupEntry& e = tab.back();
+    ARG_CHECK(q[0] + (int64_t)d.nsplit * d.Cout * d.Ktot <= slab_numel && q[8] + (int64_t)e.coutv * e.cv * e.ntaps <= dw_numel,
+              "wgrad_reduce_group: entry %d reaches past its tensor", i);
+    ds.push_back(d);
+  }
+  if (layerwise) {
+    for (const WgradSlabs& d : ds) {
+      int rc = reduce_slabs(d.slab, d.nsplit, d.Cout, d.Ktot, d.dw, d.C, d.ntaps, d.cout_valid, d.cin_valid, st);
+      if (rc) return rc;
+    }
+    return MMSKIN_OK;
+  }
+  WgradGroupEntry* dev = nullptr;
+  HIP_CHECK_RET(hipMalloc((void**)&dev, tab.size() * sizeof(WgradGroupEntry)));
+  int rc = MMSKIN_OK;
+  if (hipMemcpy(dev, tab.data(), tab.size() * sizeof(WgradGroupEntry), hipMemcpyHostToDevice) != hipSuccess) rc = MMSKIN_ERR_HIP;
+  if (!rc) rc = launch_wgrad_reduce_group(dev, n, nblocks, slabs, dw, nullptr, st);
+  if (hipStreamSynchronize(st) != hipSuccess && !rc) rc = MMSKIN_ERR_HIP;
+  (void)hipFree(dev);
+  return rc;
+}
+
 template <typename T>
 static size_t slab_bytes(int M, int Cout, int Ktot, int ntaps) {
   int BO, BKK, ns, mps;
@@ -397,16 +565,17 @@
 
 template <typename T>
 static int run_wgrad(WgradArgs& a, float* dw, int C_for_layout, int ntaps_for_layout, hipStream_t st,
-                     int cout_valid = 0, int cin_valid = 0) {
+                     int cout_valid = 0, int cin_valid = 0, WgradSlabs* defer = nullptr, bool dry = false) {
   ARG_CHECK(a.Cout % 64 == 0 && a.Ktot % 64 == 0, "wgrad: Cout=%d Ktot=%d must be multiples of 64", a.Cout, a.Ktot);
   ARG_CHECK(a.C % DT<T>::EPC == 0, "wgrad: C=%d", a.C);
   ARG_CHECK(a.OW <= 240 && a.OH <= 240, "wgrad: output %dx%d too large for the 16-bit reciprocal pixel stepping", a.OH, a.OW);
   if constexpr (sizeof(T) == 2) {
     WgradRingPlan rp;
     if (wgrad_ring_plan(a, rp)) {
-      int rc = wgrad_ring_launch(a, rp, st);
+      a.nsplit = rp.nsplit;
+      int rc = dry ? MMSKIN_OK : wgrad_ring_launch(a, rp, st);
       if (rc) return rc;
-      return reduce_slabs(a.slab, a.nsplit, a.Cout, a.Ktot, dw, C_for_layout, ntaps_for_layout, cout_valid, cin_valid, st);
+      return finish_slabs(a.slab, a.nsplit, a.Cout, a.Ktot, dw, C_for_layout, ntaps_for_layout, cout_valid, cin_valid, st, defer, dry);
     }
   }
   int BO, BKK;
@@ -416,12 +585,13 @@
   { const char* v = getenv("MMSKIN_WGRAD_ABLATE"); a.ablate = v ? atoi(v) : 0; }
 #endif
   int rc;
-  if (BO == 128 && BKK == 128) rc = launch_wg<T, 128, 128, 2>(a, st);
+  if (dry) rc = MMSKIN_OK;
+  else if (BO == 128 && BKK == 128) rc = launch_wg<T, 128, 128, 2>(a, st);
   else if (BO == 128) rc = launch_wg<T, 128, 64, 2>(a, st);
   else if (BKK == 128) rc = launch_wg<T, 64, 128, 2>(a, st);
   else rc = launch_wg<T, 64, 64, 4>(a, st);
   if (rc) return rc;
-  return reduce_slabs(a.slab, a.nsplit, a.Cout, a.Ktot, dw, C_for_layout, ntaps_for_layout, cout_valid, cin_valid, st);
+  return finish_slabs(a.slab, a.nsplit, a.Cout, a.Ktot, dw, C_for_layout, ntaps_for_layout, cout_valid, cin_valid, st, defer, dry);
 }
 
 
@@ -607,27 +777,29 @@
   return (size_t)(ns + (ns > WG_DIRECT_SPLITS ? WG_GROUPS : 0)) * s.Cout * 9 * s.Cin * sizeof(float);
 }
 static int launch_wgrad3(const ConvShape& s, Wgrad3Args& a, const bf16_t* dout, const bf16_t* in, float* slab, float* dw,
-                         hipStream_t st, int cout_valid, int cin_valid) {
+                         hipStream_t st, int cout_valid, int cin_valid, WgradSlabs* defer, bool dry) {
   a.dy = dout; a.in = in; a.slab = slab;
-  HIP_CHECK_RET(opt_in_dynamic_lds(reinterpret_cast<const void*>(wgrad3x3_kernel), W3_LDS_BYTES));
-  hipLaunchKernelGGL(wgrad3x3_kernel, dim3(a.nblk_o * a.nblk_c * a.nsplit), dim3(256), W3_LDS_BYTES, st, a);
-  HIP_CHECK_RET(hipGetLastError());
-  return reduce_slabs(slab, a.nsplit, s.Cout, 9 * s.Cin, dw, s.Cin, 9, cout_valid, cin_valid, st);
+  if (!dry) {
+    HIP_CHECK_RET(opt_in_dynamic_lds(reinterpret_cast<const void*>(wgrad3x3_kernel), W3_LDS_BYTES));
+    hipLaunchKernelGGL(wgrad3x3_kernel, dim3(a.nblk_o * a.nblk_c * a.nsplit), dim3(256), W3_LDS_BYTES, st, a);
+    HIP_CHECK_RET(hipGetLastError());
+  }
+  return finish_slabs(slab, a.nsplit, s.Cout, 9 * s.Cin, dw, s.Cin, 9, cout_valid, cin_valid, st, defer, dry);
 }
 
 template <typename T>
-int launch_conv_wgrad(const ConvShape& s, const T* dout, const T* in, float* slab, float* dw_oihw,
-                      hipStream_t st, int cout_valid, int cin_valid) {
+static int conv_wgrad_impl(const ConvShape& s, const T* dout, const T* in, float* slab, float* dw_oihw,
+                           hipStream_t st, int cout_valid, int cin_valid, WgradSlabs* defer, bool dry) {
   ARG_CHECK(s.kh * s.kw <= MMSKIN_MAX_TAPS, "wgrad: too many taps");
   if constexpr (sizeof(T) == 2) {
     int nsr = 0;
     if (wgrad3_ring_takes(s, &nsr)) {
-      int rc = launch_wgrad3_ring(s, dout, in, slab, st, &nsr);
+      int rc = dry ? MMSKIN_OK : launch_wgrad3_ring(s, dout, in, slab, st, &nsr);
       if (rc) return rc;
-      return reduce_slabs(slab, nsr, s.Cout, 9 * s.Cin, dw_oihw, s.Cin, 9, cout_valid, cin_valid, st);
+      return finish_slabs(slab, nsr, s.Cout, 9 * s.Cin, dw_oihw, s.Cin, 9, cout_valid, cin_valid, st, defer, dry);
     }
     Wgrad3Args a3 = {};
-    if (wgrad3_plan(s, a3)) return launch_wgrad3(s, a3, dout, in, slab, dw_oihw, st, cout_valid, cin_valid);
+    if (wgrad3_plan(s, a3)) return launch_wgrad3(s, a3, dout, in, slab, dw_oihw, st, cout_valid, cin_valid, defer, dry);
   }
   WgradArgs a = {};
   a.dy = dout; a.in = in; a.slab = slab;
@@ -642,12 +814,21 @@
       a.offy[r * s.kw + q] = (int8_t)(r - s.pad);
       a.offx[r * s.kw + q] = (int8_t)(q - s.pad);
     }
-  return run_wgrad<T>(a, dw_oihw, s.Cin, s.kh * s.kw, st, cout_valid, cin_valid);
-}
-
+  return run_wgrad<T>(a, dw_oihw, s.Cin, s.kh * s.kw, st, cout_valid, cin_valid, defer, dry);
+}
 template <typename T>
-int launch_stem_conv_wgrad(int N, int OH, int OW, int Hp, int Wp, const T* dout, const T* img4,
-                           float* slab, float* dwv, hipStream_t st) {
+int launch_conv_wgrad(const ConvShape& s, const T* dout, const T* in, float* slab, float* dw_oihw,
+                      hipStream_t st, int cout_valid, int cin_valid, WgradSlabs* defer) {
+  return conv_wgrad_impl<T>(s, dout, in, slab, dw_oihw, st, cout_valid, cin_valid, defer, false);
+}
+template <typename T>
+int conv_wgrad_describe(const ConvShape& s, WgradSlabs* out) {
+  return conv_wgrad_impl<T>(s, nullptr, nullptr, nullptr, nullptr, nullptr, 0, 0, out, true);
+}
+
+template <typename T>
+static int stem_wgrad_impl(int N, int OH, int OW, int Hp, int Wp, const T* dout, const T* img4,
+                           float* slab, float* dwv, hipStream_t st, WgradSlabs* defer, bool dry) {
   WgradArgs a = {};
   a.dy = dout; a.in = img4; a.slab = slab;
   a.N = N; a.IH = Hp; a.IW = Wp / 2; a.C = 32; a.Cpitch = 8;
@@ -655,7 +836,16 @@
   a.Sy = 2; a.Sx = 1; a.ntaps = 8;
   a.M = N * OH * OW;
   for (int r = 0; r < 8; ++r) { a.offy[r] = (int8_t)r; a.offx[r] = 0; }
-  return run_wgrad<T>(a, dwv, 256, 1, st);
+  return run_wgrad<T>(a, dwv, 256, 1, st, 0, 0, defer, dry);
+}
+template <typename T>
+int launch_stem_conv_wgrad(int N, int OH, int OW, int Hp, int Wp, const T* dout, const T* img4,
+                           float* slab, float* dwv, hipStream_t st, WgradSlabs* defer) {
+  return stem_wgrad_impl<T>(N, OH, OW, Hp, Wp, dout, img4, slab, dwv, st, defer, false);
+}
+template <typename T>
+int stem_wgrad_describe(int N, int OH, int OW, int Hp, int Wp, WgradSlabs* out) {
+  return stem_wgrad_impl<T>(N, OH, OW, Hp, Wp, nullptr, nullptr, nullptr, nullptr, nullptr, out, true);
 }
 
 size_t vgg_first_wgrad_slab_bytes(int N, int H, int W) {
@@ -678,7 +868,9 @@
 
 #define INST(T)                                                                                   \
   template int launch_vgg_first_conv_wgrad<T>(int, int, int, int, int, const T*, const T*, float*, float*, hipStream_t, int); \
-  template int launch_conv_wgrad<T>(const ConvShape&, const T*, const T*, float*, float*, hipStream_t, int, int); \
-  template int launch_stem_conv_wgrad<T>(int, int, int, int, int, const T*, const T*, float*, float*, hipStream_t);
+  template int launch_conv_wgrad<T>(const ConvShape&, const T*, const T*, float*, float*, hipStream_t, int, int, WgradSlabs*); \
+  template int conv_wgrad_describe<T>(const ConvShape&, WgradSlabs*);                                       \
+  template int stem_wgrad_describe<T>(int, int, int, int, int, WgradSlabs*);                                \
+  template int launch_stem_conv_wgrad<T>(int, int, int, int, int, const T*, const T*, float*, float*, hipStream_t, WgradSlabs*);
 INST(float)
 INST(bf16_t)
diff --git a/multimodal-model-skin-lesion-classifier_amd/mmskin/_lib.py b/multimodal-model-skin-lesion-classifier_amd/mmskin/_lib.py
--- a/multimodal-model-skin-lesion-classifier_amd/mmskin/_lib.py
+++ b/multimodal-model-skin-lesion-classifier_amd/mmskin/_lib.py
@@ -60,6 +60,7 @@
     "mmskin_conv2d_dgrad_fused_rows": (_i, [_i] * 9),
     "mmskin_conv2d_dgrad_fused": (_i, [_P] * 8 + [_i] * 9 + [_P, _P]),
     "mmskin_wgrad3_ring_launches": (_i64, []),
+    "mmskin_wgrad_reduce_group": (_i, [_P, _i64, _P, _i64, _i, _P, _i, _P]),
     "mmskin_abn_workspace_bytes": (_i64, [_i] * 5),
     "mmskin_abn_backward": (_i, [_P] * 6 + [_i] * 5 + [_P, _P, _P, _P]),
     "mmskin_adam_step": (_i, [_P] * 4 + [_i64] + [ctypes.c_double] * 5 + [_i64, _P]),
```

Measured after the change: 15190 images/sec. Within noise of the previous version (-0.0%).
